# gattia/pyfocusr

Measured on AMD Instinct MI355X. Metric: lowest-k eigenpairs/sec + KNN-correspondence wall-clock, 250k-vertex mesh pair k=5, higher is better.
Workload: dtype f64

## Files before the change

### include/pyfocusr_hip.h

```cpp
#ifndef PYFOCUSR_HIP_H
#define PYFOCUSR_HIP_H

#include <stddef.h>
#include <stdint.h>

#ifdef __cplusplus
extern "C" {
#endif

#define PF_VERSION 1

#define PF_OK 0
#define PF_E_ARG (-1)
#define PF_E_HIP (-2)
#define PF_E_DEGENERATE (-3)
#define PF_E_STATE (-4)
#define PF_E_PERSIST_TIMEOUT (-5)

#define PF_OP_RW 0
#define PF_OP_SYM 1

typedef struct pf_ctx pf_ctx;
typedef struct pf_graph pf_graph;
typedef struct pf_mesh pf_mesh;

typedef struct pf_graph_info {
    int64_t n;
    int64_t n_faces;
    int64_t nnz_w;
    int64_t nnz_l;
    int32_t is_symmetric;
    int32_t n_isolated;
    int32_t n_components;
    int32_t max_degree;
    int64_t sell_entries;
    int64_t n_pad;
    int64_t n_oneway;
    double spectral_bound;
} pf_graph_info;

typedef struct pf_timing {
    double op_ms;
    int64_t op_launches;
    double op_bytes;
    double knn_ms;
    double build_ms;
    double persist_ms;
    int64_t persist_launches;
    int64_t persist_steps;
    double persist_bytes;
    double persist_lds_bytes;
} pf_timing;

int pf_version(void);
const char* pf_last_error(void);
int pf_device_count(void);
int pf_create(int device, pf_ctx** out);
void pf_destroy(pf_ctx* ctx);
int pf_sync(pf_ctx* ctx);
void* pf_stream(pf_ctx* ctx);
int pf_timing_enable(pf_ctx* ctx, int on);
int pf_timing_get(pf_ctx* ctx, pf_timing* out, int reset);

int pf_graph_build(pf_ctx* ctx, const double* pts, int64_t n, const int32_t* faces, int64_t n_faces,
                   int32_t verts_per_face, pf_graph** out);
int pf_mesh_upload(pf_ctx* ctx, const double* pts, int64_t n, const int32_t* faces, int64_t n_faces,
                   int32_t verts_per_face, pf_mesh** out);
void pf_mesh_free(pf_mesh* mesh);
int pf_graph_build_device(pf_mesh* mesh, pf_graph** out);
int pf_graph_build_device2(pf_mesh* mesh_a, pf_mesh* mesh_b, pf_graph** out_a, pf_graph** out_b);
int pf_graph_from_matrix(pf_ctx* ctx, int64_t n, const int32_t* rowptr, const int32_t* colidx, const double* values,
                         pf_graph** out);
void pf_graph_free(pf_graph* g);
int pf_graph_get_info(pf_graph* g, pf_graph_info* out);
int pf_graph_download(pf_graph* g, int32_t* rowptr, int32_t* colidx, double* w, double* l_offdiag,
                      double* deg, double* l_diag, int32_t* component_label);

int pf_ws_ensure(pf_graph* g, int32_t n_slots);
int pf_ws_upload(pf_graph* g, int32_t slot, const double* x);
int pf_ws_download(pf_graph* g, int32_t first, int32_t count, double* out);
int pf_ws_copy(pf_graph* g, int32_t src, int32_t dst, int32_t count);
int pf_start_vector(pf_graph* g, int32_t slot, uint64_t seed);
int pf_mask_isolated(pf_graph* g, int32_t slot);
int pf_lock_null_vectors(pf_graph* g, int32_t op, int32_t* n_locked);

int pf_spmv(pf_graph* g, int32_t op, int32_t src, int32_t dst);
int pf_spmv_multi(pf_graph* g, int32_t op, int32_t src_first, int32_t dst_first, int32_t count);
int pf_persist_enable(int on);
int pf_persist_two_step(int level);
int pf_persist_pair_halves(int on);
int pf_persist_clock(pf_ctx* ctx, double* kernel_ms, int64_t* launches, int reset);
typedef struct pf_persist_info {
    int32_t enabled;
    int32_t two_step;
    int32_t owner;
    int32_t timeouts;
    int64_t launches;
    int64_t launches_two_step;
    int32_t suspended_for;
    int32_t rearms;
    int32_t owner_switches;
    int32_t hold_ticks;
} pf_persist_info;
int pf_persist_state(pf_ctx* ctx , pf_persist_info* out);
int pf_persist_test_hook(int n_launches);
int pf_cheb(pf_graph* g, int32_t op, int32_t src, int32_t dst, int32_t degree, double c, double e, double rho);
int pf_cheb2(pf_graph* ga, int32_t op_a, int32_t src_a, int32_t dst_a, int32_t degree_a, double c_a, double e_a, double rho_a,
             pf_graph* gb, int32_t op_b, int32_t src_b, int32_t dst_b, int32_t degree_b, double c_b, double e_b, double rho_b);
int pf_dots(pf_graph* g, int32_t w, int32_t first, int32_t count, double* out);
int pf_orth(pf_graph* g, int32_t w, int32_t first, int32_t count, double* h, double* nrm);
int pf_orth_begin(pf_graph* g, int32_t w, int32_t first, int32_t count, int32_t normalize);
int pf_orth_end(pf_graph* g, double* h, double* nrm);
int pf_orth_begin2(pf_graph* ga, int32_t w_a, int32_t first_a, int32_t count_a, int32_t normalize_a, pf_graph* gb, int32_t w_b,
                   int32_t first_b, int32_t count_b, int32_t normalize_b);
int pf_orth_cheb2(pf_graph* ga, pf_graph* gb, const int32_t* orth, const int32_t* cheb_i, const double* cheb_d);
int pf_orth_redone(pf_graph* g);
int pf_orth_strict(pf_graph* g, int32_t on);
int pf_orth_device_passes(pf_graph* g, int32_t on);
int pf_orth_split(pf_graph* g, int32_t first2, int32_t split);
int pf_orth_one_launch(int32_t on);
int pf_scale(pf_graph* g, int32_t slot, double alpha);
int pf_combine(pf_graph* g, int32_t src_first, int32_t m, const double* Y, int32_t k, int32_t dst_first);
int pf_resnorm(pf_graph* g, int32_t ax, int32_t x, double lam, double* out);
int pf_gram(pf_graph* g, int32_t first_a, int32_t count_a, int32_t first_b, int32_t count_b, double* out);
int pf_resnorms(pf_graph* g, int32_t ax_first, int32_t x_first, const double* lam, int32_t count, double* out);
int pf_finalize_vectors(pf_graph* g, int32_t first, int32_t count, int32_t from_sym, int32_t minmax,
                        double* out);
int pf_finalize_vectors_begin(pf_graph* g, int32_t first, int32_t count, int32_t from_sym, int32_t minmax, double* out);
int pf_finalize_vectors_end(pf_graph* g);
int pf_final_remap_begin(pf_graph* g, const int32_t* col, const double* sign, int32_t count, double* out);
int pf_host_alloc(size_t bytes, void** out);
int pf_host_free(void* p);
int pf_host_detach(void* p);
int pf_final_rows(pf_graph* g, const int64_t* rows, int64_t n_rows, double* out);
int pf_point_rows(pf_graph* g, const int64_t* rows, int64_t n_rows, double* out);
int pf_spmv_host(pf_graph* g, int32_t op, const double* x, double* y);
int pf_mean_filter(pf_graph* g, const double* values, int32_t ncols, int32_t iterations, double* out);

int pf_knn1(pf_ctx* ctx, const double* ref, int64_t n_ref, const double* qry, int64_t n_qry, int32_t d,
            int64_t* idx_out, double* d2_out);
int pf_knn_mode(pf_ctx* ctx, int32_t mode);
int pf_knn_tree_stats(pf_ctx* ctx, int32_t enable_counting, int64_t* leaves_scanned, int64_t* supers_opened);
int pf_knn_count(pf_ctx* ctx, int32_t enable_counting, int64_t* pairs);
int pf_knn_wave_stats(pf_ctx* ctx, double* sum_us, double* max_us, int64_t* waves, int64_t* max_candidates, double* detail);
int pf_knn(pf_ctx* ctx, const double* ref, int64_t n_ref, const double* qry, int64_t n_qry, int32_t d, int32_t k,
           int64_t* idx_out, double* d2_out);
int pf_knn1_graphs(pf_graph* ref_g, pf_graph* qry_g, int32_t d, const int32_t* col_ref, const double* scale_ref,
                   const int32_t* col_qry, const double* scale_qry, int64_t* idx_out, double* d2_out);
int pf_knn1_blocks(pf_ctx* ctx, const double* ref_block, int64_t n_ref, int32_t ref_stride, const double* qry_block,
                   int64_t n_qry, int32_t qry_stride, int32_t d, const int32_t* col_ref, const double* scale_ref,
                   const int32_t* col_qry, const double* scale_qry, int64_t* idx_out, double* d2_out);
int pf_eigsort_costs(pf_graph* g_target, pf_graph* g_source, const int64_t* rows_t, int64_t m_t, const int64_t* rows_s, int64_t m_s,
                     int32_t k, const int32_t* col_t, const double* sign_t, const int32_t* col_s, const double* sign_s, double* out,
                     int64_t* idx_out);
int pf_final_device(pf_graph* g, double** block, int64_t* n_rows, int32_t* n_cols);
int pf_knn_upload(pf_ctx* ctx, const double* ref, int64_t n_ref, const double* qry, int64_t n_qry, int32_t d);
int pf_knn_run(pf_ctx* ctx);
int pf_knn_download(pf_ctx* ctx, int64_t* idx_out, double* d2_out);

typedef struct pf_eigs_stats {
    int64_t matvecs;
    int32_t outer_steps;
    int32_t restarts;
    int32_t filter_resets;
    int32_t degree;
    int32_t n_null;
    double cut;
    double max_residual;
    int32_t second_passes;
    int32_t mode;
    int32_t local_steps;
    int32_t reserved;
} pf_eigs_stats;
int pf_eigs_smallest(pf_graph* g, int32_t n_wanted, int32_t minmax, double* vals, double* vecs, int32_t* n_out,
                     pf_eigs_stats* stats);
int pf_eigs_smallest_ex(pf_graph* g, int32_t n_wanted, int32_t minmax, int32_t async_download, double* vals, double* vecs,
                        double* residuals, int32_t* n_out, pf_eigs_stats* stats);
int pf_eigs_smallest2(pf_graph* ga, pf_graph* gb, int32_t n_wanted_a, int32_t n_wanted_b, int32_t minmax, int32_t async_download,
                      double* vals_a, double* vecs_a, double* res_a, int32_t* n_out_a, pf_eigs_stats* stats_a,
                      double* vals_b, double* vecs_b, double* res_b, int32_t* n_out_b, pf_eigs_stats* stats_b);

typedef struct pf_rows pf_rows;
int pf_op_step(pf_graph* g, int32_t op, int32_t x, int32_t prev, int32_t out, double alpha, double shift, double beta);
int pf_cheb_steps(pf_graph* g, int32_t op, int32_t prev, int32_t cur, int32_t k_first, int32_t n_steps, double c, double e,
                  double rho, int32_t* out_prev, int32_t* out_cur);
int pf_axpy(pf_graph* g, int32_t w, int32_t first, int32_t count, const double* coef);
int pf_rows_create(pf_graph* g, const int64_t* rows, int64_t n, pf_rows** out);
void pf_rows_free(pf_rows* r);
int pf_rows_gather(pf_rows* r, int32_t slot, double* out);
int pf_rows_scatter(pf_rows* r, int32_t slot, const double* in);
int pf_rows_gather_dev(pf_rows* r, int32_t slot, double* dst_device);
int pf_rows_scatter_dev(pf_rows* r, int32_t slot, const double* src_device);
int pf_rows_set_sources(pf_rows* r, const int64_t* offsets);
int pf_rows_gather2_dev(pf_rows* r, int32_t slot_a, int32_t slot_b, double* dst_device, int64_t stride);
int pf_rows_scatter2_dev(pf_rows* r, int32_t slot_a, int32_t slot_b, const double* src_device, int64_t stride);
int pf_rows_fill(pf_rows* r, int32_t slot, double value);

typedef struct pf_surface pf_surface;
int pf_surface_create(pf_ctx* ctx, const double* points, int64_t n, const int32_t* faces, int64_t n_faces,
                      int32_t verts_per_face, pf_surface** out);
void pf_surface_free(pf_surface* s);
int pf_surface_closest(pf_surface* s, const double* qry, int64_t n_qry, double* out_pts, int32_t* out_face,
                       double* out_d2);
int pf_surface_distance(pf_surface* s, const double* qry, int64_t n_qry, double* out_d2, int32_t* out_face,
                        double* stats);
int pf_surface_prepare_signed(pf_surface* s, const double* points, const int32_t* faces, int64_t* topology);
int pf_surface_signed_distance(pf_surface* s, const double* qry, int64_t n_qry, double* out_sd, int32_t* out_face,
                               int32_t* out_feature, int64_t* n_ambiguous);
int pf_surface_prepare_winding(pf_surface* s);
int pf_surface_winding(pf_surface* s, const double* qry, int64_t n_qry, double beta, double* out_w, double* out_bound);

typedef struct pf_cpd pf_cpd;
int pf_cpd_create(pf_ctx* ctx, const double* X, int64_t N, const double* Y, int64_t M, int32_t d, pf_cpd** out);
void pf_cpd_free(pf_cpd* h);
int pf_cpd_estep(pf_cpd* h, const double* TY, double sigma2, double w, double* P1, double* Pt1, double* PX);
int pf_cpd_set_basis(pf_cpd* h, const double* Q, int32_t K);
int pf_cpd_weighted_gram(pf_cpd* h, double* H);
int pf_cpd_affine_sums(pf_cpd* h, double* shifts, double* sums);
int pf_cpd_apply_affine(pf_cpd* h, const double* B, const double* t);
int pf_cpd_deform_sums(pf_cpd* h, double* H, double* R);
int pf_cpd_apply_deform(pf_cpd* h, const double* C, double* sums);
int pf_cpd_download(pf_cpd* h, double* TY, double* P1, double* Pt1, double* PX);
int pf_cpd_gram(pf_ctx* ctx, const double* A, int64_t n_a, const double* B, int64_t n_b, int32_t d, double beta,
                const double* V, int32_t n_cols, double* out);

typedef struct pf_assign_stats {
    int32_t phases;
    int32_t dense_passes;
    int64_t rounds;
    int64_t bids;
    int64_t dense_bids;
// ... 19 lines not shown
```

### pyfocusr_amd/_hip.py

```python
import atexit
import ctypes as C
import os
import threading
import weakref

import numpy as np

_HERE = os.path.dirname(os.path.abspath(__file__))
LIB_PATH = os.environ.get("PYFOCUSR_HIP_LIB", os.path.join(_HERE, "csrc", "libpyfocusr_hip.so"))

PF_OP_RW = 0
PF_OP_SYM = 1

_f64p = C.POINTER(C.c_double)
_i32p = C.POINTER(C.c_int32)
_i64p = C.POINTER(C.c_int64)


class HipUnavailable(RuntimeError):
    pass


class PfError(RuntimeError):
    def __init__(self, code, msg):
        RuntimeError.__init__(self, "libpyfocusr_hip error %d: %s" % (code, msg))
        self.code = code


class GraphInfo(C.Structure):
    _fields_ = [("n", C.c_int64), ("n_faces", C.c_int64), ("nnz_w", C.c_int64), ("nnz_l", C.c_int64),
                ("is_symmetric", C.c_int32), ("n_isolated", C.c_int32), ("n_components", C.c_int32),
                ("max_degree", C.c_int32), ("sell_entries", C.c_int64), ("n_pad", C.c_int64), ("n_oneway", C.c_int64),
                ("spectral_bound", C.c_double)]


class EigsStats(C.Structure):
    _fields_ = [("matvecs", C.c_int64), ("outer_steps", C.c_int32), ("restarts", C.c_int32), ("filter_resets", C.c_int32),
                ("degree", C.c_int32), ("n_null", C.c_int32), ("cut", C.c_double), ("max_residual", C.c_double),
                ("second_passes", C.c_int32), ("mode", C.c_int32), ("local_steps", C.c_int32), ("reserved", C.c_int32)]


class Timing(C.Structure):
    _fields_ = [("op_ms", C.c_double), ("op_launches", C.c_int64), ("op_bytes", C.c_double), ("knn_ms", C.c_double),
                ("build_ms", C.c_double), ("persist_ms", C.c_double), ("persist_launches", C.c_int64),
                ("persist_steps", C.c_int64), ("persist_bytes", C.c_double), ("persist_lds_bytes", C.c_double)]


class AssignStats(C.Structure):
    _fields_ = [("phases", C.c_int32), ("dense_passes", C.c_int32), ("rounds", C.c_int64), ("bids", C.c_int64),
                ("dense_bids", C.c_int64), ("candidate_edges", C.c_int64), ("launches", C.c_int64),
                ("device_bytes", C.c_int64), ("k", C.c_int32), ("eps_floor_hit", C.c_int32), ("eps_initial", C.c_double),
                ("eps_final", C.c_double), ("eps_floor", C.c_double), ("total_cost", C.c_double),
                ("gap_bound", C.c_double), ("lower_bound", C.c_double), ("ms_candidates", C.c_double),
                ("ms_auction", C.c_double), ("ms_certificate", C.c_double)]

    def as_dict(self):
        return {name: getattr(self, name) for name, _ in self._fields_}


SIGNATURES = {
    "pf_version": (C.c_int, []),
    "pf_last_error": (C.c_char_p, []),
    "pf_device_count": (C.c_int, []),
    "pf_create": (C.c_int, [C.c_int, C.POINTER(C.c_void_p)]),
    "pf_destroy": (None, [C.c_void_p]),
    "pf_sync": (C.c_int, [C.c_void_p]),
    "pf_stream": (C.c_void_p, [C.c_void_p]),
    "pf_timing_enable": (C.c_int, [C.c_void_p, C.c_int]),
    "pf_timing_get": (C.c_int, [C.c_void_p, C.POINTER(Timing), C.c_int]),
    "pf_graph_build": (C.c_int, [C.c_void_p, _f64p, C.c_int64, _i32p, C.c_int64, C.c_int32, C.POINTER(C.c_void_p)]),
    "pf_mesh_upload": (C.c_int, [C.c_void_p, _f64p, C.c_int64, _i32p, C.c_int64, C.c_int32, C.POINTER(C.c_void_p)]),
    "pf_mesh_free": (None, [C.c_void_p]),
    "pf_graph_build_device": (C.c_int, [C.c_void_p, C.POINTER(C.c_void_p)]),
    "pf_graph_build_device2": (C.c_int, [C.c_void_p, C.c_void_p, C.POINTER(C.c_void_p), C.POINTER(C.c_void_p)]),
    "pf_graph_from_matrix": (C.c_int, [C.c_void_p, C.c_int64, _i32p, _i32p, _f64p, C.POINTER(C.c_void_p)]),
    "pf_graph_free": (None, [C.c_void_p]),
    "pf_graph_get_info": (C.c_int, [C.c_void_p, C.POINTER(GraphInfo)]),
    "pf_graph_download": (C.c_int, [C.c_void_p, _i32p, _i32p, _f64p, _f64p, _f64p, _f64p, _i32p]),
    "pf_ws_ensure": (C.c_int, [C.c_void_p, C.c_int32]),
    "pf_ws_upload": (C.c_int, [C.c_void_p, C.c_int32, _f64p]),
    "pf_ws_download": (C.c_int, [C.c_void_p, C.c_int32, C.c_int32, _f64p]),
    "pf_ws_copy": (C.c_int, [C.c_void_p, C.c_int32, C.c_int32, C.c_int32]),
    "pf_start_vector": (C.c_int, [C.c_void_p, C.c_int32, C.c_uint64]),
    "pf_mask_isolated": (C.c_int, [C.c_void_p, C.c_int32]),
    "pf_lock_null_vectors": (C.c_int, [C.c_void_p, C.c_int32, _i32p]),
    "pf_spmv": (C.c_int, [C.c_void_p, C.c_int32, C.c_int32, C.c_int32]),
    "pf_spmv_multi": (C.c_int, [C.c_void_p, C.c_int32, C.c_int32, C.c_int32, C.c_int32]),
    "pf_knn_mode": (C.c_int, [C.c_void_p, C.c_int32]),
    "pf_knn_tree_stats": (C.c_int, [C.c_void_p, C.c_int32, C.POINTER(C.c_int64), C.POINTER(C.c_int64)]),
    "pf_persist_enable": (C.c_int, [C.c_int]),
    "pf_persist_two_step": (C.c_int, [C.c_int]),
    "pf_persist_pair_halves": (C.c_int, [C.c_int]),
    "pf_persist_clock": (C.c_int, [C.c_void_p, C.POINTER(C.c_double), C.POINTER(C.c_int64), C.c_int]),
    "pf_persist_state": (C.c_int, [C.c_void_p, C.c_void_p]),
    "pf_persist_test_hook": (C.c_int, [C.c_int]),
    "pf_cheb": (C.c_int, [C.c_void_p, C.c_int32, C.c_int32, C.c_int32, C.c_int32, C.c_double, C.c_double, C.c_double]),
    "pf_cheb2": (C.c_int, [C.c_void_p, C.c_int32, C.c_int32, C.c_int32, C.c_int32, C.c_double, C.c_double, C.c_double,
                           C.c_void_p, C.c_int32, C.c_int32, C.c_int32, C.c_int32, C.c_double, C.c_double, C.c_double]),
    "pf_dots": (C.c_int, [C.c_void_p, C.c_int32, C.c_int32, C.c_int32, _f64p]),
    "pf_orth": (C.c_int, [C.c_void_p, C.c_int32, C.c_int32, C.c_int32, _f64p, _f64p]),
    "pf_orth_begin": (C.c_int, [C.c_void_p, C.c_int32, C.c_int32, C.c_int32, C.c_int32]),
    "pf_orth_end": (C.c_int, [C.c_void_p, _f64p, _f64p]),
    "pf_orth_split": (C.c_int, [C.c_void_p, C.c_int32, C.c_int32]),
    "pf_orth_one_launch": (C.c_int, [C.c_int32]),
    "pf_orth_begin2": (C.c_int, [C.c_void_p, C.c_int32, C.c_int32, C.c_int32, C.c_int32, C.c_void_p, C.c_int32, C.c_int32, C.c_int32,
                                 C.c_int32]),
    "pf_orth_cheb2": (C.c_int, [C.c_void_p, C.c_void_p, _i32p, _i32p, _f64p]),
    "pf_eigsort_costs": (C.c_int, [C.c_void_p, C.c_void_p, _i64p, C.c_int64, _i64p, C.c_int64, C.c_int32, _i32p, _f64p, _i32p, _f64p, _f64p,
                                   _i64p]),
    "pf_orth_redone": (C.c_int, [C.c_void_p]),
    "pf_orth_strict": (C.c_int, [C.c_void_p, C.c_int32]),
    "pf_scale": (C.c_int, [C.c_void_p, C.c_int32, C.c_double]),
    "pf_combine": (C.c_int, [C.c_void_p, C.c_int32, C.c_int32, _f64p, C.c_int32, C.c_int32]),
    "pf_resnorm": (C.c_int, [C.c_void_p, C.c_int32, C.c_int32, C.c_double, _f64p]),
    "pf_gram": (C.c_int, [C.c_void_p, C.c_int32, C.c_int32, C.c_int32, C.c_int32, _f64p]),
    "pf_resnorms": (C.c_int, [C.c_void_p, C.c_int32, C.c_int32, _f64p, C.c_int32, _f64p]),
    "pf_finalize_vectors": (C.c_int, [C.c_void_p, C.c_int32, C.c_int32, C.c_int32, C.c_int32, _f64p]),
    "pf_finalize_vectors_begin": (C.c_int, [C.c_void_p, C.c_int32, C.c_int32, C.c_int32, C.c_int32, _f64p]),
    "pf_finalize_vectors_end": (C.c_int, [C.c_void_p]),
    "pf_final_remap_begin": (C.c_int, [C.c_void_p, _i32p, _f64p, C.c_int32, _f64p]),
    "pf_host_alloc": (C.c_int, [C.c_size_t, C.POINTER(C.c_void_p)]),
    "pf_host_free": (C.c_int, [C.c_void_p]),
    "pf_final_rows": (C.c_int, [C.c_void_p, _i64p, C.c_int64, _f64p]),
    "pf_point_rows": (C.c_int, [C.c_void_p, _i64p, C.c_int64, _f64p]),
    "pf_spmv_host": (C.c_int, [C.c_void_p, C.c_int32, _f64p, _f64p]),
    "pf_mean_filter": (C.c_int, [C.c_void_p, _f64p, C.c_int32, C.c_int32, _f64p]),
    "pf_knn1": (C.c_int, [C.c_void_p, _f64p, C.c_int64, _f64p, C.c_int64, C.c_int32, _i64p, _f64p]),
    "pf_knn": (C.c_int, [C.c_void_p, _f64p, C.c_int64, _f64p, C.c_int64, C.c_int32, C.c_int32, _i64p, _f64p]),
    "pf_knn1_graphs": (C.c_int, [C.c_void_p, C.c_void_p, C.c_int32, _i32p, _f64p, _i32p, _f64p, _i64p, _f64p]),
    "pf_knn1_blocks": (C.c_int, [C.c_void_p, C.c_void_p, C.c_int64, C.c_int32, C.c_void_p, C.c_int64, C.c_int32, C.c_int32,
                                 _i32p, _f64p, _i32p, _f64p, _i64p, _f64p]),
    "pf_final_device": (C.c_int, [C.c_void_p, C.POINTER(C.c_void_p), _i64p, _i32p]),
    "pf_knn_upload": (C.c_int, [C.c_void_p, _f64p, C.c_int64, _f64p, C.c_int64, C.c_int32]),
    "pf_knn_run": (C.c_int, [C.c_void_p]),
    "pf_knn_download": (C.c_int, [C.c_void_p, _i64p, _f64p]),
    "pf_eigs_smallest": (C.c_int, [C.c_void_p, C.c_int32, C.c_int32, _f64p, _f64p, C.POINTER(C.c_int32), C.POINTER(EigsStats)]),
    "pf_knn_count": (C.c_int, [C.c_void_p, C.c_int32, C.POINTER(C.c_int64)]),
    "pf_knn_wave_stats": (C.c_int, [C.c_void_p, C.POINTER(C.c_double), C.POINTER(C.c_double), C.POINTER(C.c_int64), C.POINTER(C.c_int64),
                                    _f64p]),
    "pf_host_detach": (C.c_int, [C.c_void_p]),
    "pf_orth_device_passes": (C.c_int, [C.c_void_p, C.c_int32]),
    "pf_eigs_smallest_ex": (C.c_int, [C.c_void_p, C.c_int32, C.c_int32, C.c_int32, _f64p, _f64p, _f64p, C.POINTER(C.c_int32),
                                      C.POINTER(EigsStats)]),
    "pf_eigs_smallest2": (C.c_int, [C.c_void_p, C.c_void_p, C.c_int32, C.c_int32, C.c_int32, C.c_int32,
                                    _f64p, _f64p, _f64p, C.POINTER(C.c_int32), C.POINTER(EigsStats),
                                    _f64p, _f64p, _f64p, C.POINTER(C.c_int32), C.POINTER(EigsStats)]),
    "pf_op_step": (C.c_int, [C.c_void_p, C.c_int32, C.c_int32, C.c_int32, C.c_int32, C.c_double, C.c_double, C.c_double]),
    "pf_cheb_steps": (C.c_int, [C.c_void_p, C.c_int32, C.c_int32, C.c_int32, C.c_int32, C.c_int32, C.c_double, C.c_double,
                                C.c_double, C.POINTER(C.c_int32), C.POINTER(C.c_int32)]),
    "pf_axpy": (C.c_int, [C.c_void_p, C.c_int32, C.c_int32, C.c_int32, _f64p]),
    "pf_rows_create": (C.c_int, [C.c_void_p, _i64p, C.c_int64, C.POINTER(C.c_void_p)]),
    "pf_rows_free": (None, [C.c_void_p]),
    "pf_rows_gather": (C.c_int, [C.c_void_p, C.c_int32, _f64p]),
    "pf_rows_scatter": (C.c_int, [C.c_void_p, C.c_int32, _f64p]),
    "pf_rows_gather_dev": (C.c_int, [C.c_void_p, C.c_int32, C.c_void_p]),
    "pf_rows_scatter_dev": (C.c_int, [C.c_void_p, C.c_int32, C.c_void_p]),
    "pf_rows_set_sources": (C.c_int, [C.c_void_p, _i64p]),
    "pf_rows_gather2_dev": (C.c_int, [C.c_void_p, C.c_int32, C.c_int32, C.c_void_p, C.c_int64]),
    "pf_rows_scatter2_dev": (C.c_int, [C.c_void_p, C.c_int32, C.c_int32, C.c_void_p, C.c_int64]),
    "pf_rows_fill": (C.c_int, [C.c_void_p, C.c_int32, C.c_double]),
    "pf_surface_create": (C.c_int, [C.c_void_p, _f64p, C.c_int64, _i32p, C.c_int64, C.c_int32, C.POINTER(C.c_void_p)]),
    "pf_surface_free": (None, [C.c_void_p]),
    "pf_surface_closest": (C.c_int, [C.c_void_p, _f64p, C.c_int64, _f64p, _i32p, _f64p]),
    "pf_surface_distance": (C.c_int, [C.c_void_p, _f64p, C.c_int64, _f64p, _i32p, _f64p]),
    "pf_surface_prepare_signed": (C.c_int, [C.c_void_p, _f64p, _i32p, _i64p]),
    "pf_surface_signed_distance": (C.c_int, [C.c_void_p, _f64p, C.c_int64, _f64p, _i32p, _i32p, _i64p]),
    "pf_surface_prepare_winding": (C.c_int, [C.c_void_p]),
    "pf_surface_winding": (C.c_int, [C.c_void_p, _f64p, C.c_int64, C.c_double, _f64p, _f64p]),
    "pf_cpd_create": (C.c_int, [C.c_void_p, _f64p, C.c_int64, _f64p, C.c_int64, C.c_int32, C.POINTER(C.c_void_p)]),
    "pf_cpd_free": (None, [C.c_void_p]),
    "pf_cpd_estep": (C.c_int, [C.c_void_p, _f64p, C.c_double, C.c_double, _f64p, _f64p, _f64p]),
    "pf_cpd_set_basis": (C.c_int, [C.c_void_p, _f64p, C.c_int32]),
    "pf_cpd_weighted_gram": (C.c_int, [C.c_void_p, _f64p]),
    "pf_cpd_affine_sums": (C.c_int, [C.c_void_p, _f64p, _f64p]),
    "pf_cpd_apply_affine": (C.c_int, [C.c_void_p, _f64p, _f64p]),
    "pf_cpd_deform_sums": (C.c_int, [C.c_void_p, _f64p, _f64p]),
    "pf_cpd_apply_deform": (C.c_int, [C.c_void_p, _f64p, _f64p]),
    "pf_cpd_download": (C.c_int, [C.c_void_p, _f64p, _f64p, _f64p, _f64p]),
    "pf_cpd_gram": (C.c_int, [C.c_void_p, _f64p, C.c_int64, _f64p, C.c_int64, C.c_int32, C.c_double, _f64p, C.c_int32, _f64p]),
    "pf_assign": (C.c_int, [C.c_void_p, _f64p, C.c_int64, _f64p, C.c_int64, C.c_int32, _i64p, _f64p, _f64p,
                            C.POINTER(AssignStats)]),
}

_lib = None
_lib_lock = threading.Lock()
_live_graphs = weakref.WeakSet()
_live_contexts = weakref.WeakSet()


@atexit.register
def _shutdown():
    for g in list(_live_graphs):
        g.close()
    for c in list(_live_contexts):
        c.close()


def load_library():
    global _lib
    with _lib_lock:
        if _lib is not None:
            return _lib
        if not os.path.exists(LIB_PATH):
            raise HipUnavailable(
                "%s not found: build it with `python -c 'import __graft_entry__ as g; g.build()'` "
                "(hipcc --offload-arch=gfx950); there is no CPU fallback" % LIB_PATH)
        lib = C.CDLL(LIB_PATH)
        for name, (res, args) in SIGNATURES.items():
            fn = getattr(lib, name)
            fn.restype = res
            fn.argtypes = args
        _lib = lib
        return lib


PF_E_DEGENERATE = -3
PF_E_STATE = -4
PF_E_PERSIST_TIMEOUT = -5


class _PinnedBlock(object):
    __slots__ = ("ptr", "nbytes")

    def __init__(self, ptr, nbytes):
        self.ptr, self.nbytes = ptr, nbytes

    def __del__(self):
        try:
            _pinned_release(self.ptr, self.nbytes)
        except Exception:
            pass

# ... 856 lines not shown
```

### pyfocusr_amd/csrc/pf_assemble.hip

```cpp
#include <string.h>

#include <algorithm>
#include <string>

#include "pf_internal.h"
#include "pf_launch.h"

namespace {

struct k_count_edges {
    static constexpr int BOUNDS = PF_BLOCK;
    static __device__ __forceinline__ void run(const int32_t* __restrict__ faces, int64_t n_edges,
                                                          int32_t vpf, int64_t n, int32_t* __restrict__ cnt,
                                                          int32_t* __restrict__ rank, int32_t* __restrict__ flags,
                                                          double* __restrict__ quarter) {
    const int64_t e = (int64_t)blockIdx.x * PF_BLOCK + threadIdx.x;
    if (e == 0 && quarter) *quarter = 0.25;
    if (e >= n_edges) return;
    const int64_t f = e / vpf;
    const int32_t k = (int32_t)(e - f * vpf);
    const int32_t src = faces[e];
    const int32_t dst = faces[f * vpf + (k + 1 == vpf ? 0 : k + 1)];
    if (src < 0 || src >= n || dst < 0 || dst >= n) {
        atomicOr(flags, 1);
// ... 814 lines not shown
            PF_TRY(scratch(&b_rank, n_edges));
            PF_TRY(scratch(&b_start, n + 1));
            PF_TRY(scratch(&b_rcol, n_edges));
            PF_TRY(scratch(&b_rw, n_edges));
            PF_TRY(dev_alloc(st, &g->rowptr, n + 1));
            PF_TRY(dev_alloc(st, &g->deg, 3 * g->n_pad));
            g->g = g->deg + g->n_pad;
            g->sg = g->deg + 2 * g->n_pad;
            g->deg_block = true;
            PF_TRY(dev_alloc(st, &g->diag, g->n_pad));
            PF_TRY(dev_alloc(st, &g->label, g->n_pad));
            PF_TRY(dev_alloc(st, &g->perm, g->n_pad));
            PF_TRY(dev_alloc(st, &g->iperm, g->n_pad));
            PF_TRY(dev_alloc(st, &g->smooth, g->n_pad));
            PF_TRY(dev_alloc(st, &g->slice_ptr, g->n_slices + 1));

            PF_TRY(dev_alloc(st, &g->perm_m, g->n_pad));
            PF_TRY(dev_alloc(st, &g->iperm_m, g->n_pad));
            PF_HIP(pfl::memset_words(st, zeroed, 0, sizeof(int32_t) * (size_t)(2 * zstride + 8)));
            PF_HIP(pfl::memset_words(st, g->deg, 0, sizeof(double) * 3 * g->n_pad));
            if (pos == 0) PF_HIP(pfl::event_record(st, ctx->ev0));
            PF_TRY(pf_morton_order(g, mesh->pts, robust ? nullptr : b_flags + 1));
            PF_TRY(scratch(&pts_m, 3 * n));
            PF_TRY(scratch(&faces_m, n_edges));
            d_pts = pts_m, d_faces = faces_m;
            if (n) {
                pfl::launch<k_renumber_points>(dim3(nblk(3 * n)), dim3(PF_BLOCK), 0, st, mesh->pts, g->morder, n, pts_m);
                PF_HIP(hipGetLastError());
            }
            if (n_edges) {
                pfl::launch<k_renumber_faces>(dim3(nblk(n_edges)), dim3(PF_BLOCK), 0, st, mesh->faces, g->mrank, n_edges, n, faces_m);
                PF_HIP(hipGetLastError());
            }

            if (face_bound) PF_TRY(scratch(&pmin, 1));
            if (n_edges) {
                pfl::launch<k_count_edges>(dim3(nblk(n_edges)), dim3(PF_BLOCK), 0, st, d_faces, n_edges, vpf, n, b_cnt, b_rank, b_flags, reinterpret_cast<double*>(pmin));
                PF_HIP(hipGetLastError());
            }
            PF_TRY(pf_exclusive_scan_i32(st, b_cnt, b_start, n + 1));
            if (n_edges) {
                pfl::launch<k_scatter_edges>(dim3(nblk(n_edges)), dim3(PF_BLOCK), 0, st, d_faces, d_pts, n_edges, vpf, n, b_start, b_rank, b_rcol, b_rw, b_flags);
                PF_HIP(hipGetLastError());
            }
            return PF_OK;
        }
        if (k == 1) {
            pfl::launch<k_sort_unique_rows>(dim3(nblk(n)), dim3(PF_BLOCK), 0, st, b_start, n, b_rcol, b_rw, b_ucnt, g->morder);
            PF_HIP(hipGetLastError());
            PF_TRY(pf_exclusive_scan_i32(st, b_ucnt, g->rowptr, n + 1));
            PF_TRY(dev_alloc(st, &g->col, n_edges));
            PF_TRY(dev_alloc(st, &g->w, n_edges));
            pfl::launch<k_compact_rows>(dim3(nblk(n)), dim3(PF_BLOCK), 0, st, b_start, g->rowptr, n, b_rcol, b_rw, g->col, g->w, g->deg, g->g, g->sg);
            PF_HIP(hipGetLastError());
            if (pfl::tl_rec && pf_stream_b(ctx) && ctx->fork_ev) {
                hipStream_t side = ctx->stream_b;
                hipEvent_t ev = ctx->fork_ev;
                pfl::call(st, [=](hipStream_t s) {
                    (void)hipEventRecord(ev, s);
                    (void)hipStreamWaitEvent(side, ev, 0);
                });
                g->side_stream = side;
            }
            if (face_bound) {
                pfl::launch<k_face_bound>(dim3(nblk(n_faces)), dim3(PF_BLOCK), 0, g->side_stream ? g->side_stream : st, d_faces, d_pts, n_faces, n, pmin);
                PF_HIP(hipGetLastError());
            }
            fin.g = g, fin.d_pts = d_pts, fin.numeric_symmetry = false, fin.d_extra = b_flags, fin.h_extra = h_flags;
            fin.nnz_from_rowptr = true, fin.d_pmin = pmin, fin.h_pmin = &h_pmin, fin.pos = pos;
            return PF_OK;
        }
        if (k == 2) return fin.begin_stats_and_labels();
        return fin.queue_order(false);
    }

    int end() {
        const int64_t n = mesh->n;
        PF_TRY(fin.end());
        if (h_flags[1] != 0 && !(h_flags[0] & 7)) {
            needs_robust = true;
            return PF_OK;
        }
        PF_CHECK(!(h_flags[0] & 1), PF_E_ARG, "pf_graph_build: face index out of range [0,%lld)", (long long)n);
        PF_CHECK(!(h_flags[0] & 2), PF_E_DEGENERATE, "pf_graph_build: a face repeats a vertex on one edge");
        PF_CHECK(!(h_flags[0] & 4), PF_E_DEGENERATE,
                 "pf_graph_build: an edge has zero length or non-finite coordinates (the reference would store an "
                 "infinite weight, graph.py:177-178)");
        PF_CHECK(!fin.extra_hit, PF_E_HIP, "pf_graph_build: unexpected assembly flag");
        g->spectral_bound = 2.0;
        if (pmin && g->is_symmetric && g->nnz_w == n_edges && h_pmin > 0.0 && h_pmin <= 0.25) {
            const double disc = 1.0 - 4.0 * h_pmin;
            const double b = (1.0 + (1.0 + sqrt(disc > 0.0 ? disc : 0.0)) / 2.0) * (1.0 + 1e-12);
            g->spectral_bound = b < 2.0 ? b : 2.0;
        }
        PF_TRY(dev_alloc(st, &g->pts, 3 * n));
        PF_HIP(pfl::memcpy_async(st, g->pts, mesh->pts, sizeof(double) * 3 * n, hipMemcpyDeviceToDevice));
        return PF_OK;
    }
};

}

extern "C" {

void pf_graph_free(pf_graph* g) {
    if (!g) return;
    if (!g->ctx) {
        delete g;
        return;
    }
    hipSetDevice(g->ctx->device);
    hipStream_t st = g->ctx->stream;
    (void)pf_finalize_vectors_end(g);
    {
        std::lock_guard<std::mutex> lk(g->ctx->deferred_mutex);
        auto& dq = g->ctx->deferred;
        dq.erase(std::remove(dq.begin(), dq.end(), g), dq.end());
    }
    if (g->final_stats) g->ctx->pinned_pool.emplace_back(g->final_stats_cap, reinterpret_cast<double*>(g->final_stats));
    if (g->final_ready) g->ctx->event_pool.push_back(g->final_ready);
    if (g->final_done) g->ctx->event_pool.push_back(g->final_done);
    pf_free(st, g->persist_ring);
    pf_free(st, g->persist_ring2);
    pf_free(st, g->final_vecs);
    pf_free(st, g->pts);
    pf_window_slots_free(g);
    pf_free(st, g->rowptr);
    pf_free(st, g->col);
    pf_free(st, g->w);
    pf_free(st, g->deg);
    if (!g->deg_block) {
        pf_free(st, g->g);
        pf_free(st, g->sg);
    }
    pf_free(st, g->label);
    if (g->perm_m != g->perm) pf_free(st, g->perm_m);
    if (g->iperm_m != g->iperm) pf_free(st, g->iperm_m);
    pf_free(st, g->morder);
    pf_free(st, g->mrank);
    pf_free(st, g->order_bbox);
    pf_free(st, g->perm);
    pf_free(st, g->iperm);
    pf_free(st, g->smooth);
    pf_free(st, g->stage);
    pf_free(st, g->slice_ptr);
    pf_free(st, g->scol);
    pf_free(st, g->sval_rw);
    pf_free(st, g->sval_sym);
    pf_free(st, g->diag);
    pf_free(st, g->mf_col);
    pf_free(st, g->mf_val);
    pf_free(st, g->ws);
    pf_free(st, g->partials);
    pf_free(st, g->coef);
    pf_free(st, g->orth_counter);
    if (g->orth_pending >= 0 || g->small_pending > 0 || g->px_state == -2) pfl::sync(st);
    if (g->orth_host) g->ctx->pinned_pool.emplace_back(g->orth_host_cap, g->orth_host);
    if (g->orth_ev) g->ctx->event_pool.push_back(g->orth_ev);
    if (g->px_host) g->ctx->pinned_pool.emplace_back(g->px_host_cap, g->px_host);
    if (g->px_ev) g->ctx->event_pool.push_back(g->px_ev);
    if (g->small_host) g->ctx->pinned_pool.emplace_back(g->small_host_cap, g->small_host);
    if (g->small_ev) g->ctx->event_pool.push_back(g->small_ev);
    delete g;
}


int pf_mesh_upload(pf_ctx* ctx, const double* pts, int64_t n, const int32_t* faces, int64_t n_faces, int32_t vpf,
                   pf_mesh** out) {
    PF_CHECK(ctx && pts && out && (faces || n_faces == 0), PF_E_ARG, "pf_mesh_upload: NULL argument");
    PF_CHECK(n > 0 && n < (int64_t)1 << 31, PF_E_ARG, "pf_mesh_upload: n = %lld out of range", (long long)n);
    PF_CHECK(n_faces >= 0 && vpf >= 2 && n_faces * vpf < (int64_t)1 << 31, PF_E_ARG,
             "pf_mesh_upload: faces %lld x %d out of range", (long long)n_faces, vpf);
    *out = nullptr;
    PF_HIP(hipSetDevice(ctx->device));
    pf_mesh* m = new pf_mesh();
    m->ctx = ctx;
    m->n = n;
    m->n_faces = n_faces;
    m->vpf = vpf;
    hipStream_t st = ctx->stream;
    int r = dev_alloc(st, &m->pts, 3 * n);
    if (r == PF_OK) r = dev_alloc(st, &m->faces, n_faces * vpf);
    hipError_t e = hipSuccess;
    if (r == PF_OK) e = pfl::memcpy_async(ctx->stream, m->pts, pts, sizeof(double) * 3 * n, hipMemcpyHostToDevice);
    if (r == PF_OK && e == hipSuccess && n_faces)
        e = pfl::memcpy_async(ctx->stream, m->faces, faces, sizeof(int32_t) * n_faces * vpf, hipMemcpyHostToDevice);
    if (r == PF_OK && e == hipSuccess) e = pfl::sync(ctx->stream);
    if (r != PF_OK || e != hipSuccess) {
        if (e != hipSuccess) pf_set_error("pf_mesh_upload: %s", hipGetErrorString(e));
        pf_mesh_free(m);
        return r != PF_OK ? r : PF_E_HIP;
    }
    *out = m;
    return PF_OK;
}

void pf_mesh_free(pf_mesh* m) {
    if (!m) return;
    pf_free(m->ctx->stream, m->pts);
    pf_free(m->ctx->stream, m->faces);
    delete m;
}

int pf_graph_build(pf_ctx* ctx, const double* pts, int64_t n, const int32_t* faces, int64_t n_faces,
                   int32_t vpf, pf_graph** out) {
    PF_CHECK(out != nullptr, PF_E_ARG, "pf_graph_build: out is NULL");
    *out = nullptr;
    pf_mesh* m = nullptr;
    PF_TRY(pf_mesh_upload(ctx, pts, n, faces, n_faces, vpf, &m));
    int r = pf_graph_build_device(m, out);
    pf_mesh_free(m);
    return r;
}

int pf_graph_build_device(pf_mesh* mesh, pf_graph** out) {
    PF_CHECK(mesh && out, PF_E_ARG, "pf_graph_build_device: NULL argument");
    pf_ctx* ctx = mesh->ctx;
    *out = nullptr;
    PF_HIP(hipSetDevice(ctx->device));
    MeshBuild job;
    PF_TRY(job.begin(mesh));
    PF_TRY(job.end());
    if (job.needs_robust) {
        if (getenv("PF_DEBUG_WINDOWS")) fprintf(stderr, "pyfocusr_hip: renumbering by counting gave up, building again with the general sort\n");
        MeshBuild again;
        again.robust = true;
        PF_TRY(again.begin(mesh));
        PF_TRY(again.end());
        PF_HIP(pfl::sync(ctx->stream));
        again.ok = true;
        *out = again.g;
        return PF_OK;
    }
    PF_HIP(pfl::event_record(ctx->stream, ctx->ev1));
    ctx->build_pending = true;
    if (pf_persist_enabled()) PF_TRY(pf_window_slots_begin(job.g));
    job.ok = true;
    *out = job.g;
    return PF_OK;
}

int pf_graph_build_device2(pf_mesh* mesh_a, pf_mesh* mesh_b, pf_graph** out_a, pf_graph** out_b) {
    PF_CHECK(mesh_a && mesh_b && out_a && out_b, PF_E_ARG, "pf_graph_build_device2: NULL argument");
    PF_CHECK(mesh_a->ctx == mesh_b->ctx, PF_E_ARG, "pf_graph_build_device2: the two meshes must belong to one ctx");
    pf_ctx* ctx = mesh_a->ctx;
    *out_a = *out_b = nullptr;
    PF_HIP(hipSetDevice(ctx->device));
    if (!pf_stream_b(ctx)) {
        PF_TRY(pf_graph_build_device(mesh_a, out_a));
        const int r = pf_graph_build_device(mesh_b, out_b);
        if (r != PF_OK) {
            pf_graph_free(*out_a);
            *out_a = nullptr;
        }
        return r;
    }
    hipStream_t st = ctx->stream;
    bool redo = false;
    {
        MeshBuild a, b;
        pfl::Recorder ra, rb;
        struct Unhook {
            ~Unhook() { pfl::tl_rec = nullptr; }
        } unhook;
        int rc = a.prepare(mesh_a, 0);
        if (rc == PF_OK) rc = b.prepare(mesh_b, 1);
        for (int k = 0; k < MeshBuild::N_PHASES && rc == PF_OK; ++k) {
            pfl::tl_rec = &ra;
            rc = a.phase(k);
            pfl::tl_rec = &rb;
            if (rc == PF_OK) rc = b.phase(k);
            pfl::tl_rec = nullptr;
            pfl::flush(ra, &rb);
        }
        if (rc == PF_OK) {
            pfl::tl_rec = &ra;
            rc = a.end();
            pfl::tl_rec = &rb;
            if (rc == PF_OK) rc = b.end();
            if (rc == PF_OK && !(a.needs_robust || b.needs_robust) && pf_persist_enabled()) {
                pfl::tl_rec = &ra;
                rc = pf_window_slots_begin(a.g);
                pfl::tl_rec = &rb;
                if (rc == PF_OK) rc = pf_window_slots_begin(b.g);
            }
        }
        pfl::tl_rec = nullptr;
        pfl::flush(ra, &rb);
        if (rc != PF_OK) {
            (void)pfl::sync(ctx->stream_b);
            (void)pfl::sync(st);
        }
        a.release();
        b.release();
        if (rc == PF_OK) {
            const hipError_t e1 = hipEventRecord(ctx->ev1, st);
            if (e1 == hipSuccess) ctx->build_pending = true;
            else rc = PF_E_HIP, pf_set_error("pf_graph_build_device2: %s", hipGetErrorString(e1));
        }
        if (rc != PF_OK) return rc;
        if (a.needs_robust || b.needs_robust) {
            redo = true;
        } else {
            a.ok = b.ok = true;
            *out_a = a.g;
            *out_b = b.g;
// ... 208 lines not shown
```

### pyfocusr_amd/csrc/pf_eigs.hip

```cpp
#include <math.h>

#include <algorithm>
#include <vector>

#include "pf_internal.h"
#include "pf_krylov.h"

namespace {

struct DeviceOps final : pfk::Ops {
    pf_graph* g;
    explicit DeviceOps(pf_graph* graph) : g(graph) {}
    int64_t n() const override { return g->n; }
    int64_t n_isolated() const override { return g->n_isolated; }
    int32_t n_components() const override { return g->n_components; }
    int32_t n_oneway() const override { return g->n_oneway; }
    bool symmetric() const override { return g->is_symmetric; }
    double spectral_bound() const override { return g->spectral_bound; }
    int ws_ensure(int32_t slots) override { return pf_ws_ensure(g, slots); }
    int lock_nulls(int32_t op, int32_t* locked) override { return pf_lock_null_vectors(g, op, locked); }
    int orth_strict(bool on) override { return pf_orth_strict(g, on ? 1 : 0); }
    int orth_always_twice(bool on, bool strict_otherwise) override { return pf_orth_strict(g, on ? 2 : (strict_otherwise ? 1 : 0)); }
    int orth_device_passes(bool on) override { return pf_orth_device_passes(g, on ? 1 : 0); }
    int start_vector(int32_t slot, uint64_t seed) override { return pf_start_vector(g, slot, seed); }
    int orth_begin(int32_t w, int32_t first, int32_t count) override { return pf_orth_begin(g, w, first, count, 1); }
    int orth_end(double* h, double* nrm, bool* redone) override {
        PF_TRY(pf_orth_end(g, h, nrm));
        const int r = pf_orth_redone(g);
        *redone = r == 1;
        last_twice = r == 2;
        return PF_OK;
    }
    int cheb(int32_t op, int32_t src, int32_t dst, int32_t degree, double c, double e, double rho) override {
        return pf_cheb(g, op, src, dst, degree, c, e, rho);
    }
    int combine(int32_t src_first, int32_t m, const double* Y, int32_t k, int32_t dst_first) override {
        return pf_combine(g, src_first, m, Y, k, dst_first);
    }
    int combine2(int32_t src_first, int32_t m, const double* Y, int32_t k, int32_t dst_first, int32_t src_first2, int32_t dst_first2) override {
        return pf_combine2(g, src_first, m, Y, k, dst_first, src_first2, dst_first2);
    }
    int copy(int32_t src, int32_t dst, int32_t count) override { return pf_ws_copy(g, src, dst, count); }
    int spmv_multi(int32_t op, int32_t src_first, int32_t dst_first, int32_t count) override {
        return pf_spmv_multi(g, op, src_first, dst_first, count);
    }
    int gram(int32_t first_a, int32_t count_a, int32_t first_b, int32_t count_b, double* out) override {
        return pf_gram(g, first_a, count_a, first_b, count_b, out);
    }
    int resnorms(int32_t ax_first, int32_t x_first, const double* lam, int32_t count, double* out) override {
        return pf_resnorms(g, ax_first, x_first, lam, count, out);
    }
    int gram_begin(int32_t first_a, int32_t count_a, int32_t first_b, int32_t count_b, bool self_b) override {
        PF_TRY(pf_gram_begin(g, first_a, count_a, first_b, count_b, 0));
        return self_b ? pf_gram_begin(g, first_b, count_b, first_b, count_b, 1) : PF_OK;
    }
    bool orth_split(int32_t first2, int32_t split) override { return pf_orth_split(g, first2, split) == PF_OK; }
    int gram_end(double* out) override { return pf_small_end(g, out); }
    int resnorms_begin(int32_t ax_first, int32_t x_first, const double* lam, int32_t count) override {
        return pf_resnorms_begin(g, ax_first, x_first, lam, count);
    }
    int resnorms_end(double* out) override { return pf_small_end(g, out); }
    int orth_begin_pair(pfk::Ops& other, const int32_t* o) override {
        return pf_orth_begin2(g, o[0], o[1], o[2], o[3], static_cast<DeviceOps&>(other).g, o[4], o[5], o[6], o[7]);
    }
    int cheb_pair(pfk::Ops& other, const int32_t* ci, const double* cd) override {
        return pf_cheb2(g, ci[0], ci[1], ci[2], ci[3], cd[0], cd[1], cd[2], static_cast<DeviceOps&>(other).g, ci[4], ci[5], ci[6], ci[7], cd[3],
                        cd[4], cd[5]);
    }
    int orth_cheb_pair(pfk::Ops& other, const int32_t* orth, const int32_t* ci, const double* cd) override {
        return pf_orth_cheb2(g, static_cast<DeviceOps&>(other).g, orth, ci, cd);
    }
};

int ellipse_hint() {
    const char* ev = getenv("PF_EIGS_ELLIPSE");
    return ev ? atoi(ev) : -1;
}

void give_up(pf_graph* g) {
    if (!g) return;
    if (g->orth_pending >= 0) {
        std::vector<double> h((size_t)g->orth_pending + 1);
        double nrm = 0.0;
        (void)pf_orth_end(g, h.data(), &nrm);
    }
    if (g->small_pending > 0) {
        (void)hipEventSynchronize(g->small_ev);
        g->small_pending = 0;
    }
    (void)pf_download_cancel(g);
}

int finish(pf_graph* g, pfk::Solver& s, int32_t minmax, double* vals, double* vecs, double* residuals, int32_t* n_out, pf_eigs_stats* stats,
           bool async) {
    *n_out = s.n_out;
    for (int i = 0; i < s.n_out; ++i) {
        vals[i] = s.vals[(size_t)i];
        if (residuals) residuals[i] = s.residuals[(size_t)i];
    }
    if (stats) *stats = s.st;
    if (s.n_out > 0) {
        PF_TRY(pf_finalize_vectors_begin(g, s.first_slot, s.n_out, s.sym ? 1 : 0, minmax ? 1 : 0, vecs));
        if (!async) PF_TRY(pf_finalize_vectors_end(g));
    }
    return PF_OK;
}

}

extern "C" int pf_eigs_smallest_ex(pf_graph* g, int32_t n_wanted, int32_t minmax, int32_t async_download, double* vals, double* vecs,
                                   double* residuals, int32_t* n_out, pf_eigs_stats* stats_out) {
    PF_CHECK(g && vals && vecs && n_out && n_wanted >= 1, PF_E_ARG, "pf_eigs_smallest: bad argument");
    int rc = PF_OK;
    for (int attempt = 0; attempt < 3; ++attempt) {
        DeviceOps ops(g);
        pfk::Solver s;
        *n_out = 0;
        rc = s.init(&ops, n_wanted, ellipse_hint());
        if (rc == PF_OK) rc = pfk::drive_single(s);
        if (rc == PF_OK) rc = pf_sync(g->ctx);
        if (rc == PF_OK) rc = finish(g, s, minmax, vals, vecs, residuals, n_out, stats_out, async_download != 0);
        if (rc != PF_OK) give_up(g);
        if (rc != PF_E_PERSIST_TIMEOUT) break;
    }
    return rc;
}

extern "C" int pf_eigs_smallest(pf_graph* g, int32_t n_wanted, int32_t minmax, double* vals, double* vecs, int32_t* n_out,
                                pf_eigs_stats* stats_out) {
    return pf_eigs_smallest_ex(g, n_wanted, minmax, 0, vals, vecs, nullptr, n_out, stats_out);
}

extern "C" int pf_eigs_smallest2(pf_graph* ga, pf_graph* gb, int32_t n_wanted_a, int32_t n_wanted_b, int32_t minmax, int32_t async_download,
                                 double* vals_a, double* vecs_a, double* res_a, int32_t* n_out_a, pf_eigs_stats* stats_a,
                                 double* vals_b, double* vecs_b, double* res_b, int32_t* n_out_b, pf_eigs_stats* stats_b) {
    PF_CHECK(ga && gb && ga != gb && vals_a && vecs_a && n_out_a && vals_b && vecs_b && n_out_b && n_wanted_a >= 1 && n_wanted_b >= 1,
             PF_E_ARG, "pf_eigs_smallest2: bad argument");
    PF_CHECK(ga->ctx == gb->ctx, PF_E_ARG, "pf_eigs_smallest2: the two graphs must share one ctx (stream)");
    int rc = PF_OK;
    for (int attempt = 0; attempt < 3; ++attempt) {
        DeviceOps oa(ga), ob(gb);
        pfk::Solver a, b;
        *n_out_a = *n_out_b = 0;
        rc = a.init(&oa, n_wanted_a, ellipse_hint());
        if (rc == PF_OK) rc = b.init(&ob, n_wanted_b, ellipse_hint());
        if (rc == PF_OK) rc = pfk::drive_pair(a, b);
        if (rc == PF_OK) rc = pf_sync(ga->ctx);
        if (rc == PF_OK) rc = finish(ga, a, minmax, vals_a, vecs_a, res_a, n_out_a, stats_a, async_download != 0);
        if (rc == PF_OK) rc = finish(gb, b, minmax, vals_b, vecs_b, res_b, n_out_b, stats_b, async_download != 0);
        if (rc != PF_OK) {
            give_up(ga);
            give_up(gb);
        }
        if (rc != PF_E_PERSIST_TIMEOUT) break;
    }
    return rc;
}
```

### pyfocusr_amd/csrc/pf_internal.h

```cpp
#pragma once
#include <hip/hip_runtime.h>
#include <stdint.h>
#include <atomic>
#include <map>
#include <mutex>
#include <unordered_map>
#include <vector>

#include "../../include/pyfocusr_hip.h"

void pf_set_error(const char* fmt, ...);

#define PF_HIP(call)                                                                          \
    do {                                                                                      \
        hipError_t e_ = (call);                                                               \
        if (e_ != hipSuccess) {                                                               \
            pf_set_error("%s:%d %s: %s", __FILE__, __LINE__, #call, hipGetErrorString(e_));   \
            (void)hipGetLastError();  \
            return PF_E_HIP;                                                                  \
        }                                                                                     \
    } while (0)

#define PF_CHECK(cond, code, ...)        \
    do {                                 \
// ... 36 lines not shown

struct pf_ctx {
    int device = 0;
    hipStream_t stream = nullptr;
    void* stage_ring = nullptr;
    hipEvent_t stage_ev[8] = {nullptr, nullptr, nullptr, nullptr, nullptr, nullptr, nullptr, nullptr};
    int stage_next = 0;
    hipStream_t copy_stream = nullptr;
    hipEvent_t ev0 = nullptr, ev1 = nullptr;
    bool timing = false;
    int timing_stride = 1;
    int64_t timing_count = 0;
    uint32_t* persist_sync = nullptr;
    int32_t* persist_abort = nullptr;
    void* persist_cal = nullptr;
    double op_ms = 0.0;
    int64_t op_launches = 0;
    double op_bytes = 0.0;
    double persist_ms = 0.0, persist_bytes = 0.0, persist_lds_bytes = 0.0;
    int64_t persist_launches = 0, persist_steps = 0;
    double knn_ms = 0.0;
    double build_ms = 0.0;
    bool build_pending = false;
    double* knn_ref = nullptr;
    double* knn_qry = nullptr;
    double* knn_ref_s = nullptr;
    double* knn_ref_soa = nullptr;
    int64_t knn_cap_ref_soa = 0, knn_ref_ld = 0;
    double* knn_qry_s = nullptr;
    unsigned* knn_ref_key = nullptr;
    unsigned* knn_qry_key = nullptr;
    int32_t* knn_cell_start = nullptr;
    int64_t knn_cap_cell = 0;
    int knn_res = 0;
    void* knn_grid = nullptr;
    int32_t* knn_ref_orig = nullptr;
    int32_t* knn_qry_orig = nullptr;
    unsigned long long* knn_ext = nullptr;
    int64_t knn_nref = 0, knn_nqry = 0;
    int64_t knn_cap_ref = 0, knn_cap_qry = 0, knn_cap_ref_s = 0, knn_cap_qry_s = 0, knn_cap_ref_key = 0,
            knn_cap_qry_key = 0, knn_cap_ref_orig = 0, knn_cap_qry_orig = 0, knn_cap_idx = 0, knn_cap_d2 = 0;
    int32_t knn_d = 0;
    int32_t knn_k = 1, knn_k_next = 1;
    int64_t* knn_idx = nullptr;
    double* knn_d2 = nullptr;
    bool knn_ready = false, knn_done = false;
    pf_knn_tree knn_tree;
    bool knn_count_on = false;
    unsigned long long* knn_visited = nullptr;
    size_t knn_visited_words = 0;
    int64_t knn_visited_waves = 0;
    int32_t knn_mode = 0;
    struct TimedSpan {
        hipEvent_t e0, e1;
        int64_t launches;
        double bytes;
        int64_t persist_steps;
        double lds_bytes;
    };
    std::vector<TimedSpan> spans_pending;
    std::vector<std::pair<hipEvent_t, hipEvent_t>> spans_free;
    std::vector<std::pair<int32_t, double*>> pinned_pool;
    void* pinned_scratch = nullptr;
    size_t pinned_scratch_bytes = 0;
    std::vector<hipEvent_t> event_pool;
    std::multimap<size_t, void*> free_blocks;
    std::unordered_map<void*, size_t> live_blocks;
    std::mutex alloc_mutex;
    hipStream_t stream_b = nullptr;
    hipEvent_t join_ev = nullptr, fork_ev = nullptr;
    std::vector<pf_graph*> deferred;
    std::mutex deferred_mutex;
    int64_t alloc_misses = 0;
    void* pinned_scratch_b = nullptr;
    size_t pinned_scratch_b_bytes = 0;
    void* pinned_scratch_knn = nullptr;
    size_t pinned_scratch_knn_bytes = 0;
};

inline uint64_t pf_next_uid() {
    static std::atomic<uint64_t> next{1};
    return next.fetch_add(1);
}

struct pf_graph {
    hipStream_t side_stream = nullptr;
    uint64_t uid = pf_next_uid();
    pf_ctx* ctx = nullptr;
    int64_t n = 0, n_pad = 0, n_faces = 0;
    int32_t vpf = 0;
    int32_t* rowptr = nullptr;
    int32_t* col = nullptr;
    double* w = nullptr;
    int64_t nnz_w = 0;
    double* deg = nullptr;
    double* g = nullptr;
    double* sg = nullptr;
    int32_t* label = nullptr;
    int32_t* morder = nullptr;
    int32_t* mrank = nullptr;
    int32_t* perm_m = nullptr;
    int32_t* iperm_m = nullptr;
    int32_t* perm = nullptr;
    int32_t* iperm = nullptr;
    unsigned long long* order_bbox = nullptr;
    double* smooth = nullptr;
    double* stage = nullptr;
    int64_t stage_cap = 0;
    int64_t n_slices = 0, sell_entries = 0;
    int64_t* slice_ptr = nullptr;
    int32_t* scol = nullptr;
    double* sval_rw = nullptr;
    double* sval_sym = nullptr;
    double* diag = nullptr;
    int32_t* mf_col = nullptr;
    double* mf_val = nullptr;
    int32_t win_rows = 1024;
    std::vector<int64_t> h_slice_ptr;
    int32_t px_state = -1;
    double* px_host = nullptr;
    int32_t px_host_cap = 0;
    hipEvent_t px_ev = nullptr;
    int32_t* px_slot = nullptr;
    int32_t* px_gh_cnt = nullptr;
    int32_t* px_gh_row = nullptr;
    int32_t* px_need = nullptr;
    std::vector<int32_t> h_px_gh_cnt;
    int64_t px_gh_total = 0;
    double* persist_ring = nullptr;
    int32_t persist_phase = 0;
    uint64_t persist_epoch = 0;
    int32_t px2_state = -1;
    int32_t* px_gh_cnt2 = nullptr;
    int32_t* px_need2 = nullptr;
    uint8_t* px_g1_w = nullptr;
    int32_t* px_g1_pos = nullptr;
    uint16_t* px_g1_slot = nullptr;
    int32_t* px_g1_gw = nullptr;
    std::vector<int32_t> h_px_gh_cnt2, h_px_g1_gw;
    int64_t px_gh2_total = 0, px_g1_entries = 0;
    int32_t single_applications = 0;
    uint64_t lds_need_partner = 0;
    int64_t lds_need_value = -2, lds_need2_value = -2;
    double* persist_ring2 = nullptr;
    int32_t persist_phase2 = 0;
    uint64_t persist_epoch2 = 0;
    int32_t is_symmetric = 0, n_isolated = 0, n_components = 0, max_degree = 0, n_oneway = 0;
    int32_t unit_g = 0;
    std::vector<int32_t> roots;
    double* ws = nullptr;
    int32_t n_slots = 0;
    double* partials = nullptr;
    int32_t partial_cap = 0;
    double* coef = nullptr;
    int32_t coef_cap = 0;
    int64_t n_chunks = 0;
    double* orth_host = nullptr;
    int32_t orth_host_cap = 0;
    int32_t orth_pending = -1;
    hipEvent_t orth_ev = nullptr;
    double* small_host = nullptr;
    int32_t small_host_cap = 0, small_pending = 0;
    bool small_root = false;
    hipEvent_t small_ev = nullptr;
    hipEvent_t orth_wait = nullptr;
    int32_t orth_w = 0, orth_first = 0, orth_normalize = 0;
    int32_t orth_redone = 0;
    double orth_serial = 0.0;
    unsigned long long* orth_counter = nullptr;
    unsigned long long orth_arrivals = 0;
    uint64_t orth_epoch = 0;
    int32_t orth_split = -1, orth_first2 = 0;
    int32_t orth_split_now = -1, orth_first2_now = 0;
    double orth_ticket = 0.0;
    double orth_thresh = 0.09;
    int32_t orth_device_passes = 0;
    int32_t orth_twice = 0;
    double* final_vecs = nullptr;
    int32_t final_count = 0;
    int32_t final_pending = 0;
    double* final_params = nullptr;
    void* final_stats = nullptr;
    int32_t final_stats_cap = 0;
    hipEvent_t final_ready = nullptr, final_done = nullptr;
    const double* dl_src = nullptr;
    double* dl_dst = nullptr;
    size_t dl_bytes = 0;
    int32_t final_check = 0;
    double* final_tmp = nullptr;
    double* pts = nullptr;
    bool deg_block = false;
    double spectral_bound = 2.0;
};

int pf_timing_collect(pf_ctx* c);
hipError_t pf_malloc(hipStream_t st, void** p, size_t bytes);
int pf_pinned_scratch(pf_ctx* c, size_t bytes, void** out, int which = 0);
int pf_copy_by_kernel(hipStream_t st, const void* src, void* dst, size_t bytes);
int pf_downloads_release(pf_ctx* c);
int pf_download_cancel(pf_graph* g);
hipStream_t pf_stream_b(pf_ctx* c);
hipError_t pf_create_side_stream(hipStream_t* s, bool low = false);
void pf_free(hipStream_t st, void* p);

__host__ __device__ static inline int64_t pf_sell_index(int64_t base, int32_t width, int32_t j, int lane) {
    const int32_t pairs = width >> 1;
    return j < 2 * pairs ? base + (int64_t)(j >> 1) * (2 * PF_WAVE) + 2 * lane + (j & 1)
                         : base + (int64_t)pairs * (2 * PF_WAVE) + lane;
}

static inline double* pf_slot(pf_graph* g, int32_t s) { return g->ws + (int64_t)s * g->n_pad; }
static inline double* pf_tmp(pf_graph* g, int which) { return g->ws + (int64_t)(g->n_slots + which) * g->n_pad; }

int pf_exclusive_scan_i32(hipStream_t st, const int32_t* in, int32_t* out, int64_t n);
int pf_exclusive_scan_i64(hipStream_t st, const int64_t* in, int64_t* out, int64_t n);

int pf_reduce_ensure(pf_graph* g, int32_t count);

int pf_compute_order(pf_graph* g, const double* d_pts, int32_t* d_overflow = nullptr);
int pf_morton_order(pf_graph* g, const double* d_pts, int32_t* d_overflow);

static inline int32_t pf_window_rows(int64_t n_pad) { return n_pad <= 262144 ? 1024 : (n_pad <= 524288 ? 2048 : 4096); }

constexpr int PF_KNN_TREE_MIN_D = 7;
int pf_knn_tree_run(pf_ctx* c);

int pf_gram_begin(pf_graph* g, int32_t first_a, int32_t count_a, int32_t first_b, int32_t count_b, int32_t append);
int pf_resnorms_begin(pf_graph* g, int32_t ax_first, int32_t x_first, const double* lam, int32_t count);
int pf_small_end(pf_graph* g, double* out);
int pf_combine2(pf_graph* g, int32_t src_first, int32_t m, const double* Y, int32_t k, int32_t dst_first, int32_t src_first2,
                int32_t dst_first2);

struct pf_persist_args {
    pf_graph* g;
    const double* vals;
    const double* src;
    double* dst;
    int32_t degree;
    double c, e, rho;
};
int pf_persist_cheb(const pf_persist_args* a, const pf_persist_args* b , int* done, double* lds_bytes ,
                    bool first_try = true );
int pf_persist_check(pf_ctx* ctx);
int pf_persist_set(int on);
void pf_persist_release(pf_ctx* ctx);
int pf_window_slots_prepare(pf_graph* g);
int pf_window_slots_begin(pf_graph* g);
bool pf_persist_enabled();
bool pf_persist_trusted();
uint64_t pf_persist_abort_epoch();
int pf_persist_sync_ensure(pf_ctx* ctx);
int pf_window_rings_prepare(pf_graph* g);
void pf_window_slots_free(pf_graph* g);
```

### pyfocusr_amd/csrc/pf_operator.hip

```cpp
#include <math.h>
#include <stdlib.h>
#include <string.h>

#include <algorithm>
#include <atomic>
#include <map>
#include <mutex>
#include <vector>

#include "pf_internal.h"

namespace {

inline unsigned nblk(int64_t n) { return (unsigned)((n + PF_BLOCK - 1) / PF_BLOCK); }

#ifndef PF_OP_BLOCK
#define PF_OP_BLOCK 256
#endif
struct OpArgs {
    const int64_t* slice_ptr;
    const int32_t* scol;
    const double* sval;
    const double* diag;
    const double* x;
// ... 388 lines not shown
                           (unsigned long long)__double_as_longlong(p), __ATOMIC_RELAXED, __HIP_MEMORY_SCOPE_AGENT);
        asm volatile("s_waitcnt vmcnt(0)" ::: "memory");
    }
    __syncthreads();
    if (threadIdx.x == 0) s_ok = orth_meet(a, a.target);
    __syncthreads();
    if (!s_ok) return;
    {
        const int b0 = threadIdx.x / PF_WAVE, b1 = b0 + PF_BLOCK / PF_WAVE;
        double s0 = 0.0, s1 = 0.0;
        for (int64_t k = lane; k < a.n_chunks; k += PF_WAVE) {
            const double x0 = b0 < count + 1 ? __longlong_as_double((long long)__hip_atomic_load(
                                                   reinterpret_cast<unsigned long long*>(a.partial) + (int64_t)b0 * a.n_chunks + k, __ATOMIC_RELAXED,
                                                   __HIP_MEMORY_SCOPE_AGENT))
                                             : 0.0;
            const double x1 = b1 < count + 1 ? __longlong_as_double((long long)__hip_atomic_load(
                                                   reinterpret_cast<unsigned long long*>(a.partial) + (int64_t)b1 * a.n_chunks + k, __ATOMIC_RELAXED,
                                                   __HIP_MEMORY_SCOPE_AGENT))
                                             : 0.0;
            s0 += x0;
            s1 += x1;
        }
#pragma unroll
        for (int off = PF_WAVE / 2; off > 0; off >>= 1) {
            s0 += __shfl_down(s0, off, PF_WAVE);
            s1 += __shfl_down(s1, off, PF_WAVE);
        }
        if (lane == 0 && b0 < count + 1) hs[b0] = s0;
        if (lane == 0 && b1 < count + 1) hs[b1] = s1;
    }
    __syncthreads();
    if (threadIdx.x == 0) {
        double sum = 0.0;
        for (int b = 0; b < count; ++b) sum += hs[b] * hs[b];
        const double before = hs[count], after = before - sum;
        int fine = after >= a.thresh * before ? 1 : 0;
        asm volatile("" : "+v"(fine));
        s_redo = fine ? 0.0 : 1.0;
        s_after = after;
        s_scale = (fine && a.normalize && after > 1e-280) ? 1.0 / sqrt(after) : 1.0;
    }
    __syncthreads();
    if (chunk == 0) {
        for (int b = threadIdx.x; b < count; b += PF_BLOCK) {
            a.hsum[b] = hs[b];
            a.host_out[b] = hs[b];
        }
        if (threadIdx.x == 0) {
            *a.nrm2 = s_after;
            a.host_out[count] = s_after;
            a.host_out[count + 1] = s_redo;
        }
        __threadfence_system();
        __syncthreads();
        if (threadIdx.x == 0) __hip_atomic_store(a.host_out + count + 2, a.ticket, __ATOMIC_RELEASE, __HIP_MEMORY_SCOPE_SYSTEM);
    }
    const double sc = s_scale;
#pragma unroll
    for (int it = 0; it < PAIRS; ++it) {
        double2 acc = cs[it];
#pragma unroll
        for (int u = 0; u < PF_ORTH_LOCAL_MAX; ++u) {
            if (u >= count) continue;
            const double hb = hs[u];
            acc.x -= hb * xs[u][it].x;
            acc.y -= hb * xs[u][it].y;
        }
        acc.x *= sc;
        acc.y *= sc;
        *reinterpret_cast<double2*>(w + lo + 2 * threadIdx.x + (int64_t)it * (2 * PF_BLOCK)) = acc;
    }
}
__global__ __launch_bounds__(PF_BLOCK) void k_scale_finishing(double* __restrict__ x, int64_t n_pad, const double* __restrict__ partial,
                                                              int64_t n_chunks, int normalize, const double* __restrict__ hsum,
                                                              int32_t count, double* __restrict__ nrm2, double* __restrict__ host_out) {
    __shared__ double s_v;
    if (threadIdx.x < PF_WAVE) {
        double s = 0.0;
        for (int64_t k = threadIdx.x; k < n_chunks; k += PF_WAVE) s += partial[k];
#pragma unroll
        for (int off = PF_WAVE / 2; off > 0; off >>= 1) s += __shfl_down(s, off, PF_WAVE);
        if (threadIdx.x == 0) s_v = s;
    }
    __syncthreads();
    const double v = s_v;
    if (blockIdx.x == 0) {
        for (int b = threadIdx.x; b < count; b += PF_BLOCK) host_out[b] = hsum[b];
        if (threadIdx.x == 0) {
            *nrm2 = v;
            host_out[count] = v;
            host_out[count + 1] = 0.0;
        }
    }
    const int64_t i = (int64_t)blockIdx.x * PF_BLOCK + threadIdx.x;
    if (normalize && i < n_pad && v > 1e-280) x[i] *= 1.0 / sqrt(v);
}

__global__ __launch_bounds__(PF_BLOCK) void k_scale(double* __restrict__ x, int64_t n_pad, double alpha) {
    const int64_t i = (int64_t)blockIdx.x * PF_BLOCK + threadIdx.x;
    if (i < n_pad) x[i] *= alpha;
}

__global__ __launch_bounds__(PF_BLOCK) void k_scale_rsqrt(double* __restrict__ x, int64_t n_pad, const double* __restrict__ nrm2) {
    const int64_t i = (int64_t)blockIdx.x * PF_BLOCK + threadIdx.x;
    const double v = *nrm2;
    if (i < n_pad && v > 1e-280) x[i] *= 1.0 / sqrt(v);
}

__global__ __launch_bounds__(PF_BLOCK) void k_mask_isolated(double* __restrict__ x, const int32_t* __restrict__ rowptr,
                                                            const int32_t* __restrict__ perm, int64_t n) {
    const int64_t r = (int64_t)blockIdx.x * PF_BLOCK + threadIdx.x;
    if (r >= n) return;
    const int32_t i = perm[r];
    if (rowptr[i + 1] == rowptr[i]) x[r] = 0.0;
}

__global__ __launch_bounds__(PF_BLOCK) void k_start_vector(double* __restrict__ x, const double* __restrict__ smooth,
                                                           const int32_t* __restrict__ perm, const int32_t* __restrict__ perm_m,
                                                           const int32_t* __restrict__ rowptr,
                                                           int64_t n_pad, unsigned long long seed, double noise) {
    const int64_t r = (int64_t)blockIdx.x * PF_BLOCK + threadIdx.x;
    if (r >= n_pad) return;
    const int32_t i = perm[r];
    const int32_t m = perm_m[r];
    double v = 0.0;
    if (i >= 0 && rowptr[m + 1] > rowptr[m]) {
        unsigned long long z = seed + 0x9E3779B97F4A7C15ull * (unsigned long long)(i + 1);
        z = (z ^ (z >> 30)) * 0xBF58476D1CE4E5B9ull;
        z = (z ^ (z >> 27)) * 0x94D049BB133111EBull;
        z ^= z >> 31;
        const double u = (double)(z >> 11) * (1.0 / 9007199254740992.0) - 0.5;
        v = smooth[r] + noise * u;
    }
    x[r] = v;
}

__global__ __launch_bounds__(PF_BLOCK) void k_permute_in(const double* __restrict__ src_old, const int32_t* __restrict__ perm,
                                                         int64_t n_pad, double* __restrict__ dst_new) {
    const int64_t r = (int64_t)blockIdx.x * PF_BLOCK + threadIdx.x;
    if (r >= n_pad) return;
    const int32_t i = perm[r];
    dst_new[r] = i >= 0 ? src_old[i] : 0.0;
}

__global__ __launch_bounds__(PF_BLOCK) void k_permute_out(const double* __restrict__ ws, int64_t n_pad, int32_t first,
                                                          int32_t count, const int32_t* __restrict__ iperm, int64_t n,
                                                          double* __restrict__ dst_old ) {
    const int64_t i = (int64_t)blockIdx.x * PF_BLOCK + threadIdx.x;
    if (i >= n) return;
    const int64_t r = iperm[i];
    for (int c = 0; c < count; ++c) dst_old[(int64_t)c * n + i] = ws[(int64_t)(first + c) * n_pad + r];
}

__global__ __launch_bounds__(PF_BLOCK) void k_null_vector(double* __restrict__ x, const int32_t* __restrict__ label,
                                                          const int32_t* __restrict__ rowptr,
                                                          const double* __restrict__ deg, const int32_t* __restrict__ perm,
                                                          int64_t n_pad, int32_t root, int32_t sym) {
    const int64_t r = (int64_t)blockIdx.x * PF_BLOCK + threadIdx.x;
    if (r >= n_pad) return;
    const int32_t i = perm[r];
    double v = 0.0;
    if (i >= 0 && label[i] == root && rowptr[i + 1] > rowptr[i]) v = sym ? sqrt(deg[i] + 1e-8) : 1.0;
    x[r] = v;
}

constexpr int COMBINE_COLS = 8;
__global__ __launch_bounds__(PF_BLOCK) void k_combine(double* __restrict__ ws, int64_t n_pad, int32_t src_first, int32_t m,
                                                      const double* __restrict__ Y, int32_t k, int32_t c0, int32_t ncols,
                                                      int32_t dst_first, int32_t src_first2, int32_t dst_first2) {
    const int64_t i = (int64_t)blockIdx.x * PF_BLOCK + threadIdx.x;
    if (i >= n_pad) return;
    if (blockIdx.y) src_first = src_first2, dst_first = dst_first2;
    double acc[COMBINE_COLS];
#pragma unroll
    for (int c = 0; c < COMBINE_COLS; ++c) acc[c] = 0.0;
    for (int b = 0; b < m; ++b) {
        const double v = ws[(int64_t)(src_first + b) * n_pad + i];
        const double* yr = Y + (int64_t)b * k + c0;
#pragma unroll
        for (int c = 0; c < COMBINE_COLS; ++c)
            if (c < ncols) acc[c] += v * yr[c];
    }
#pragma unroll
    for (int c = 0; c < COMBINE_COLS; ++c)
        if (c < ncols) ws[(int64_t)(dst_first + c0 + c) * n_pad + i] = acc[c];
}

__global__ __launch_bounds__(PF_BLOCK) void k_resnorm_partial(const double* __restrict__ ax, const double* __restrict__ x,
                                                              double lam, int64_t n_pad, int64_t n_chunks,
                                                              double* __restrict__ partial) {
    __shared__ double red[PF_BLOCK / PF_WAVE];
    const int64_t lo = (int64_t)blockIdx.x * PF_DOT_CHUNK;
    const int64_t hi = lo + PF_DOT_CHUNK < n_pad ? lo + PF_DOT_CHUNK : n_pad;
    double s = 0.0;
    for (int64_t i = lo + threadIdx.x; i < hi; i += PF_BLOCK) {
        const double r = ax[i] - lam * x[i];
        s += r * r;
    }
#pragma unroll
    for (int off = PF_WAVE / 2; off > 0; off >>= 1) s += __shfl_down(s, off, PF_WAVE);
    if ((threadIdx.x & (PF_WAVE - 1)) == 0) red[threadIdx.x / PF_WAVE] = s;
    __syncthreads();
    if (threadIdx.x == 0) partial[blockIdx.x] = (red[0] + red[1]) + (red[2] + red[3]);
}

__global__ __launch_bounds__(PF_BLOCK) void k_gram_partial(const double* __restrict__ ws, int64_t n_pad, int32_t first_a, int32_t first_b,
                                                           int32_t count_b, int64_t n_chunks, double* __restrict__ partial) {
    __shared__ double red[PF_BLOCK / PF_WAVE];
    const int p = blockIdx.y;
    const int i = p / count_b, j = p - i * count_b;
    const double* v = ws + (int64_t)(first_b + j) * n_pad;
    const double* w = ws + (int64_t)(first_a + i) * n_pad;
    const int64_t lo = (int64_t)blockIdx.x * PF_DOT_CHUNK;
    const int64_t hi = lo + PF_DOT_CHUNK < n_pad ? lo + PF_DOT_CHUNK : n_pad;
    double s = 0.0;
    for (int64_t r = lo + 2 * threadIdx.x; r < hi; r += 2 * PF_BLOCK) {
        const double2 a = *reinterpret_cast<const double2*>(v + r);
        const double2 c = *reinterpret_cast<const double2*>(w + r);
        s += a.x * c.x;
        s += a.y * c.y;
    }
#pragma unroll
    for (int off = PF_WAVE / 2; off > 0; off >>= 1) s += __shfl_down(s, off, PF_WAVE);
    if ((threadIdx.x & (PF_WAVE - 1)) == 0) red[threadIdx.x / PF_WAVE] = s;
    __syncthreads();
    if (threadIdx.x == 0) partial[(int64_t)p * n_chunks + blockIdx.x] = (red[0] + red[1]) + (red[2] + red[3]);
}

constexpr int PF_RESNORMS_MAX = 64;
struct LamArgs {
    double lam[PF_RESNORMS_MAX];
};
__global__ __launch_bounds__(PF_BLOCK) void k_resnorms_partial(const double* __restrict__ ws, int64_t n_pad, int32_t ax_first,
                                                               int32_t x_first, LamArgs la, int64_t n_chunks,
                                                               double* __restrict__ partial) {
    __shared__ double red[PF_BLOCK / PF_WAVE];
    const int b = blockIdx.y;
    const double* ax = ws + (int64_t)(ax_first + b) * n_pad;
    const double* x = ws + (int64_t)(x_first + b) * n_pad;
    const double lam = la.lam[b];
    const int64_t lo = (int64_t)blockIdx.x * PF_DOT_CHUNK;
    const int64_t hi = lo + PF_DOT_CHUNK < n_pad ? lo + PF_DOT_CHUNK : n_pad;
    double s = 0.0;
    for (int64_t i = lo + threadIdx.x; i < hi; i += PF_BLOCK) {
        const double r = ax[i] - lam * x[i];
        s += r * r;
    }
#pragma unroll
    for (int off = PF_WAVE / 2; off > 0; off >>= 1) s += __shfl_down(s, off, PF_WAVE);
    if ((threadIdx.x & (PF_WAVE - 1)) == 0) red[threadIdx.x / PF_WAVE] = s;
    __syncthreads();
    if (threadIdx.x == 0) partial[(int64_t)b * n_chunks + blockIdx.x] = (red[0] + red[1]) + (red[2] + red[3]);
}

struct VecStats {
    double sumsq, vmin, vmax, absmax, at_absmax;
    int64_t arg;
};

__device__ __forceinline__ void stats_merge(VecStats& a, const VecStats& b) {
    a.sumsq += b.sumsq;
    a.vmin = fmin(a.vmin, b.vmin);
    a.vmax = fmax(a.vmax, b.vmax);
    if (b.absmax > a.absmax || (b.absmax == a.absmax && b.arg < a.arg)) {
        a.absmax = b.absmax;
        a.at_absmax = b.at_absmax;
        a.arg = b.arg;
    }
}

__device__ __forceinline__ VecStats stats_shfl(const VecStats& v, int off) {
    VecStats o;
    o.sumsq = __shfl_down(v.sumsq, off, PF_WAVE);
    o.vmin = __shfl_down(v.vmin, off, PF_WAVE);
    o.vmax = __shfl_down(v.vmax, off, PF_WAVE);
    o.absmax = __shfl_down(v.absmax, off, PF_WAVE);
    o.at_absmax = __shfl_down(v.at_absmax, off, PF_WAVE);
    o.arg = __shfl_down(v.arg, off, PF_WAVE);
    return o;
}

__global__ __launch_bounds__(PF_BLOCK) void k_vec_stats_partial(const double* __restrict__ ws, int64_t n_pad, int64_t n,
                                                                int32_t first, const double* __restrict__ sg,
                                                                const int32_t* __restrict__ perm, const int32_t* __restrict__ perm_m,
                                                                int32_t from_sym, int64_t n_chunks, VecStats* __restrict__ partial) {
    __shared__ VecStats red[PF_BLOCK / PF_WAVE];
    const int b = blockIdx.y;
    const double* x = ws + (int64_t)(first + b) * n_pad;
    const int64_t lo = (int64_t)blockIdx.x * PF_DOT_CHUNK;
    const int64_t hi0 = lo + PF_DOT_CHUNK;
    const int64_t hi = hi0 < n ? hi0 : n;
    VecStats st{0.0, INFINITY, -INFINITY, -1.0, 0.0, (int64_t)1 << 62};
    for (int64_t r = lo + threadIdx.x; r < hi; r += PF_BLOCK) {
        const int64_t i = perm[r];
        double v = x[r];
        if (from_sym) v *= sg[perm_m[r]];
        VecStats e{v * v, v, v, fabs(v), v, i};
        stats_merge(st, e);
    }
#pragma unroll
    for (int off = PF_WAVE / 2; off > 0; off >>= 1) {
        VecStats o = stats_shfl(st, off);
        stats_merge(st, o);
    }
    if ((threadIdx.x & (PF_WAVE - 1)) == 0) red[threadIdx.x / PF_WAVE] = st;
    __syncthreads();
    if (threadIdx.x == 0) {
        VecStats t = red[0];
        stats_merge(t, red[1]);
        stats_merge(t, red[2]);
        stats_merge(t, red[3]);
        partial[(int64_t)b * n_chunks + blockIdx.x] = t;
    }
}

__global__ __launch_bounds__(PF_WAVE) void k_vec_stats_finish(const VecStats* __restrict__ partial, int64_t n_chunks,
                                                              VecStats* __restrict__ out) {
    const int b = blockIdx.x;
    VecStats st{0.0, INFINITY, -INFINITY, -1.0, 0.0, (int64_t)1 << 62};
    for (int64_t k = threadIdx.x; k < n_chunks; k += PF_WAVE) stats_merge(st, partial[(int64_t)b * n_chunks + k]);
#pragma unroll
    for (int off = PF_WAVE / 2; off > 0; off >>= 1) {
        VecStats o = stats_shfl(st, off);
        stats_merge(st, o);
    }
    if (threadIdx.x == 0) out[b] = st;
}

__global__ void k_vec_params(const VecStats* __restrict__ fin, int32_t count, int32_t minmax, double* __restrict__ params) {
    for (int c = threadIdx.x; c < count; c += blockDim.x) {
        const VecStats s = fin[c];
        const double sgn = s.at_absmax < 0.0 ? -1.0 : 1.0;
        const double scale = sgn / sqrt(s.sumsq);
        const double vmin = (sgn > 0 ? s.vmin : s.vmax) * scale;
        const double vmax = (sgn > 0 ? s.vmax : s.vmin) * scale;
        params[4 * c + 0] = scale;
        params[4 * c + 1] = minmax ? vmin : 0.0;
        params[4 * c + 2] = minmax ? (vmax - vmin) : 0.0;
        params[4 * c + 3] = minmax ? 0.5 : 0.0;
    }
}

__global__ __launch_bounds__(PF_BLOCK) void k_vec_apply(const double* __restrict__ ws, int64_t n_pad, int64_t n,
                                                        int32_t first, int32_t count, const double* __restrict__ sg,
                                                        const int32_t* __restrict__ iperm, const int32_t* __restrict__ mrank,
                                                        int32_t from_sym, const double* __restrict__ params, double* __restrict__ out) {
    const int64_t i = (int64_t)blockIdx.x * PF_BLOCK + threadIdx.x;
    if (i >= n) return;
    const int64_t r = iperm[i];
    const double s = from_sym ? sg[mrank ? mrank[i] : i] : 1.0;
    for (int c = 0; c < count; ++c) {
        const double scale = params[4 * c + 0], off = params[4 * c + 1], ptp = params[4 * c + 2], half = params[4 * c + 3];
        double v = (ws[(int64_t)(first + c) * n_pad + r] * s) * scale;
        if (ptp != 0.0) v = (v - off) / ptp - half;
        out[i * count + c] = v;
    }
}

__global__ __launch_bounds__(PF_BLOCK) void k_final_rows(const double* __restrict__ fin, const int64_t* __restrict__ rows, int64_t n_rows,
                                                         int32_t fc, double* __restrict__ out) {
    const int64_t e = (int64_t)blockIdx.x * PF_BLOCK + threadIdx.x;
    if (e >= n_rows * fc) return;
    const int64_t t = e / fc;
    out[e] = fin[rows[t] * fc + (e - t * fc)];
}

__global__ __launch_bounds__(PF_BLOCK) void k_fill_mean_filter(const int32_t* __restrict__ rowptr, const int32_t* __restrict__ col,
                                                               const double* __restrict__ w, const double* __restrict__ deg,
                                                               const int32_t* __restrict__ perm, const int32_t* __restrict__ iperm,
                                                               const int32_t* __restrict__ key, int64_t n_pad,
                                                               const int64_t* __restrict__ slice_ptr,
                                                               int32_t* __restrict__ mf_col, double* __restrict__ mf_val) {
    const int64_t row = (int64_t)blockIdx.x * PF_BLOCK + threadIdx.x;
    if (row >= n_pad) return;
    const int64_t s = row / PF_WAVE;
    const int lane = (int)(row & (PF_WAVE - 1));
    const int32_t width = (int32_t)((slice_ptr[s + 1] - slice_ptr[s]) / PF_WAVE) + 1;
    const int64_t base = slice_ptr[s] + (int64_t)PF_WAVE * s;
    const int32_t i = perm[row];
    int32_t e = 0;
    if (i >= 0) {
        const double dinv = 1.0 / (1.0 + deg[i]);
        bool diag_done = false;
        const int32_t ki = key ? key[i] : i;
        for (int32_t a = rowptr[i + 1] - 1; a >= rowptr[i]; --a) {
            const int32_t j = col[a];
            if (!diag_done && (key ? key[j] : j) < ki) {
                mf_col[base + (int64_t)PF_WAVE * e + lane] = (int32_t)row;
                mf_val[base + (int64_t)PF_WAVE * e + lane] = dinv;
                ++e;
                diag_done = true;
            }
            mf_col[base + (int64_t)PF_WAVE * e + lane] = iperm[j];
            mf_val[base + (int64_t)PF_WAVE * e + lane] = dinv * w[a];
            ++e;
        }
        if (!diag_done) {
            mf_col[base + (int64_t)PF_WAVE * e + lane] = (int32_t)row;
            mf_val[base + (int64_t)PF_WAVE * e + lane] = dinv;
            ++e;
        }
    }
    for (; e < width; ++e) {
        mf_col[base + (int64_t)PF_WAVE * e + lane] = (int32_t)row;
        mf_val[base + (int64_t)PF_WAVE * e + lane] = 0.0;
    }
}

template <int NC>
__global__ __launch_bounds__(PF_BLOCK) void k_mean_filter(const int64_t* __restrict__ slice_ptr, const int32_t* __restrict__ mf_col,
                                                          const double* __restrict__ mf_val, const int32_t* __restrict__ perm,
                                                          int64_t n_pad, int32_t ncols, const double* __restrict__ in,
                                                          double* __restrict__ out) {
    const int64_t row = (int64_t)blockIdx.x * PF_BLOCK + threadIdx.x;
    if (row >= n_pad) return;
    const int64_t s = row / PF_WAVE;
    const int lane = (int)(row & (PF_WAVE - 1));
    const int32_t width = (int32_t)((slice_ptr[s + 1] - slice_ptr[s]) / PF_WAVE) + 1;
    const int64_t base = slice_ptr[s] + (int64_t)PF_WAVE * s + lane;
    const bool real = perm[row] >= 0;
    if constexpr (NC > 0) {
        double acc[NC];
#pragma unroll
        for (int c = 0; c < NC; ++c) acc[c] = 0.0;
        for (int32_t e = 0; e < width; ++e) {
            const int64_t j = mf_col[base + (int64_t)PF_WAVE * e];
            const double v = mf_val[base + (int64_t)PF_WAVE * e];
            if (v != 0.0 || j != row) {
#pragma unroll
                for (int c = 0; c < NC; ++c) acc[c] += v * in[j * NC + c];
            }
        }
#pragma unroll
        for (int c = 0; c < NC; ++c) out[row * NC + c] = real ? acc[c] : 0.0;
    } else {
        for (int32_t c = 0; c < ncols; ++c) {
            double acc = 0.0;
            for (int32_t e = 0; e < width; ++e) {
                const double v = mf_val[base + (int64_t)PF_WAVE * e];
                const int64_t j = mf_col[base + (int64_t)PF_WAVE * e];
                if (v != 0.0 || j != row) acc += v * in[j * ncols + c];
            }
            out[row * ncols + c] = real ? acc : 0.0;
        }
    }
}

__global__ __launch_bounds__(PF_BLOCK) void k_rows_in(const double* __restrict__ src, const int32_t* __restrict__ perm, int64_t n_pad,
                                                      int32_t ncols, double* __restrict__ dst) {
    const int64_t t = (int64_t)blockIdx.x * PF_BLOCK + threadIdx.x;
    if (t >= n_pad * ncols) return;
    const int64_t row = t / ncols;
    const int32_t old = perm[row];
    dst[t] = old >= 0 ? src[(int64_t)old * ncols + (t - row * ncols)] : 0.0;
}
__global__ __launch_bounds__(PF_BLOCK) void k_rows_out(const double* __restrict__ src, const int32_t* __restrict__ iperm, int64_t n,
                                                       int32_t ncols, double* __restrict__ dst) {
    const int64_t t = (int64_t)blockIdx.x * PF_BLOCK + threadIdx.x;
    if (t >= n * ncols) return;
    const int64_t old = t / ncols;
    dst[t] = src[(int64_t)iperm[old] * ncols + (t - old * ncols)];
}

__global__ __launch_bounds__(PF_BLOCK) void k_rows_to_new(const int64_t* __restrict__ old_idx, const int32_t* __restrict__ iperm,
                                                          int64_t cnt, int32_t* __restrict__ new_idx) {
    const int64_t t = (int64_t)blockIdx.x * PF_BLOCK + threadIdx.x;
    if (t < cnt) new_idx[t] = iperm[old_idx[t]];
}
__global__ __launch_bounds__(PF_BLOCK) void k_rows_gather(const double* __restrict__ x, const int32_t* __restrict__ idx, int64_t cnt,
                                                          double* __restrict__ out) {
    const int64_t t = (int64_t)blockIdx.x * PF_BLOCK + threadIdx.x;
    if (t < cnt) out[t] = x[idx[t]];
}
__global__ __launch_bounds__(PF_BLOCK) void k_rows_scatter(double* __restrict__ x, const int32_t* __restrict__ idx, int64_t cnt,
                                                           const double* __restrict__ in) {
    const int64_t t = (int64_t)blockIdx.x * PF_BLOCK + threadIdx.x;
    if (t < cnt) x[idx[t]] = in[t];
}
__global__ __launch_bounds__(PF_BLOCK) void k_rows_gather2(const double* __restrict__ xa, const double* __restrict__ xb,
                                                           const int32_t* __restrict__ idx, int64_t cnt, int64_t stride,
                                                           double* __restrict__ out) {
    const int64_t t = (int64_t)blockIdx.x * PF_BLOCK + threadIdx.x;
    if (t >= cnt) return;
    const int32_t r = idx[t];
    out[t] = xa[r];
    if (xb) out[stride + t] = xb[r];
}
__global__ __launch_bounds__(PF_BLOCK) void k_rows_scatter2(double* __restrict__ xa, double* __restrict__ xb,
                                                            const int32_t* __restrict__ idx, const int64_t* __restrict__ off,
                                                            int64_t cnt, int64_t stride, const double* __restrict__ src) {
    const int64_t t = (int64_t)blockIdx.x * PF_BLOCK + threadIdx.x;
    if (t >= cnt) return;
    const int32_t r = idx[t];
    const int64_t o = off[t];
    xa[r] = src[o];
    if (xb) xb[r] = src[o + stride];
}
__global__ __launch_bounds__(PF_BLOCK) void k_rows_fill(double* __restrict__ x, const int32_t* __restrict__ idx, int64_t cnt,
                                                        double value) {
    const int64_t t = (int64_t)blockIdx.x * PF_BLOCK + threadIdx.x;
    if (t < cnt) x[idx[t]] = value;
}

int stage_ensure(pf_graph* g, int64_t elems) {
    if (elems <= g->stage_cap) return PF_OK;
    pf_free(g->ctx->stream, g->stage);
    g->stage = nullptr;
    g->stage_cap = 0;
    PF_HIP(pf_malloc(g->ctx->stream, (void**)&g->stage, sizeof(double) * (size_t)elems));
    g->stage_cap = elems;
    return PF_OK;
}

int check_slots(pf_graph* g, int32_t first, int32_t count, const char* who) {
    PF_CHECK(g != nullptr, PF_E_ARG, "%s: graph is NULL", who);
    PF_HIP(hipSetDevice(g->ctx->device));
    PF_CHECK(first >= 0 && count >= 0 && first + count <= g->n_slots, PF_E_ARG, "%s: slots [%d,%d) outside workspace of %d",
             who, first, first + count, g->n_slots);
    return PF_OK;
}

const double* op_values(pf_graph* g, int32_t op) {
    if (op == PF_OP_RW) return g->sval_rw;
    if (op == PF_OP_SYM) return g->sval_sym;
    return nullptr;
}

OpArgs op_args(pf_graph* g, const double* vals, const double* x, const double* prev, double* out, double alpha, double shift,
               double beta) {
    return OpArgs{g->slice_ptr, g->scol, vals, g->diag, x, prev, out, alpha, shift, beta, (unsigned)(g->n_pad / PF_OP_BLOCK)};
}

int64_t op_bytes(const pf_graph* g) {
    return 12 * (g->nnz_w + g->n - g->n_isolated) + 20 * g->n + 4;
}

int launch_op(pf_graph* g, const double* vals, const double* x, const double* prev, double* out, double alpha, double shift,
              double beta) {
    hipStream_t st = g->ctx->stream;
    const OpArgs a = op_args(g, vals, x, prev, out, alpha, shift, beta);
    if (prev)
        k_sell_op<true><<<a.n_blocks, PF_OP_BLOCK, 0, st>>>(a);
    else
        k_sell_op<false><<<a.n_blocks, PF_OP_BLOCK, 0, st>>>(a);
    PF_HIP(hipGetLastError());
    return PF_OK;
}

int launch_op2(pf_graph* ga, const OpArgs& a, const OpArgs& b, bool has_prev) {
    hipStream_t st = ga->ctx->stream;
    if (has_prev)
        k_sell_op2<true><<<a.n_blocks + b.n_blocks, PF_OP_BLOCK, 0, st>>>(a, b);
    else
        k_sell_op2<false><<<a.n_blocks + b.n_blocks, PF_OP_BLOCK, 0, st>>>(a, b);
    PF_HIP(hipGetLastError());
    return PF_OK;
}

struct ChebRun {
    pf_graph* g;
    const double* vals;
    const double* src;
    double* dst;
    int32_t degree;
    double c, e, rho;
    const double* yp = nullptr;
    const double* yc = nullptr;
    int32_t done = 0;

    int32_t left() const { return degree - done; }
    double* free_tmp(int which) const {
        for (int t = 0; t < PF_WS_TMPS; ++t) {
            double* b = pf_tmp(g, t);
            if (b != yp && b != yc && which-- == 0) return b;
        }
        return nullptr;
    }
    OpArgs first() {
        double* target = degree == 1 ? dst : pf_tmp(g, 0);
        const OpArgs a = op_args(g, vals, src, nullptr, target, 1.0 / (e * rho), c, 0.0);
        yp = src, yc = target, done = 1;
        return a;
    }
    OpArgs single() {
        double* target = left() == 1 ? dst : free_tmp(0);
        const OpArgs a = op_args(g, vals, yc, yp, target, 2.0 / (e * rho), c, 1.0 / (rho * rho));
        yp = yc, yc = target, done += 1;
        return a;
    }
};

struct OpTimer {
    pf_ctx* c;
    int64_t launches;
    double bytes;
    bool on;
    int64_t persist_steps = 0;
    double lds_bytes = 0.0;
    hipEvent_t e0 = nullptr, e1 = nullptr;
    OpTimer(pf_ctx* ctx, int64_t n, double b) : c(ctx), launches(n), bytes(b), on(ctx->timing) {
        if (on && ctx->timing_stride > 1) on = (ctx->timing_count++ % ctx->timing_stride) == 0;
        if (!on) return;
        if (c->spans_pending.size() >= 4096) (void)pf_timing_collect(c);
        if (!c->spans_free.empty()) {
            e0 = c->spans_free.back().first;
            e1 = c->spans_free.back().second;
            c->spans_free.pop_back();
        } else if (hipEventCreate(&e0) != hipSuccess || hipEventCreate(&e1) != hipSuccess) {
            on = false;
            return;
        }
        hipEventRecord(e0, c->stream);
    }
    int finish() {
        if (!on) return PF_OK;
        PF_HIP(hipEventRecord(e1, c->stream));
        c->spans_pending.push_back({e0, e1, launches, bytes, persist_steps, lds_bytes});
        return PF_OK;
    }
};

int small_to_host(pf_graph* g, const double* d_src, double* out, size_t count) {
    pf_ctx* c = g->ctx;
    hipStream_t st = c->stream;
    const size_t bytes = sizeof(double) * count;
    void* pin = nullptr;
    if (bytes <= ((size_t)1 << 16) && pf_pinned_scratch(c, bytes, &pin) == PF_OK) {
        PF_TRY(pf_copy_by_kernel(st, d_src, pin, bytes));
        PF_HIP(hipStreamSynchronize(st));
        memcpy(out, pin, bytes);
        return PF_OK;
    }
    PF_HIP(hipMemcpyAsync(out, d_src, bytes, hipMemcpyDeviceToHost, st));
    PF_HIP(hipStreamSynchronize(st));
    return PF_OK;
}

int dots_device(pf_graph* g, int32_t w, int32_t first, int32_t count, double* d_out, double* d_acc, int accumulate) {
    hipStream_t st = g->ctx->stream;
    PF_TRY(pf_reduce_ensure(g, count));
    dim3 grid((unsigned)g->n_chunks, (unsigned)count);
    k_dot_partial<<<grid, PF_BLOCK, 0, st>>>(g->ws, g->n_pad, first, w, g->n_chunks, g->partials);
    PF_HIP(hipGetLastError());
    k_dot_finish<<<(unsigned)count, PF_WAVE, 0, st>>>(g->partials, g->n_chunks, d_out, d_acc, accumulate);
    PF_HIP(hipGetLastError());
    return PF_OK;
}

}

int pf_reduce_ensure(pf_graph* g, int32_t count) {
    if (count > g->partial_cap) {
        pf_free(g->ctx->stream, g->partials);
        g->partials = nullptr;
        const int32_t cap = std::max(count, 64);
        PF_HIP(pf_malloc(g->ctx->stream, (void**)&g->partials, sizeof(VecStats) * (size_t)cap * (size_t)(g->n_chunks + 1)));
        g->partial_cap = cap;
    }
    if (count > g->coef_cap) {
        pf_free(g->ctx->stream, g->coef);
        g->coef = nullptr;
        const int32_t cap = std::max(count, 64);
        PF_HIP(pf_malloc(g->ctx->stream, (void**)&g->coef, sizeof(double) * 8 * (size_t)cap));
        g->coef_cap = cap;
    }
    return PF_OK;
}

extern "C" {

int pf_ws_ensure(pf_graph* g, int32_t n_slots) {
    PF_CHECK(g != nullptr && n_slots > 0, PF_E_ARG, "pf_ws_ensure: bad argument");
    if (n_slots <= g->n_slots) return PF_OK;
    PF_HIP(hipSetDevice(g->ctx->device));
    hipStream_t st = g->ctx->stream;
    double* nw = nullptr;
    const size_t bytes = sizeof(double) * (size_t)(n_slots + PF_WS_TMPS) * (size_t)g->n_pad;
    PF_HIP(pf_malloc(st, (void**)&nw, bytes));
    PF_HIP(hipMemsetAsync(nw, 0, bytes, st));
    if (g->ws && g->n_slots > 0)
        PF_HIP(hipMemcpyAsync(nw, g->ws, sizeof(double) * (size_t)g->n_slots * g->n_pad, hipMemcpyDeviceToDevice, st));
    pf_free(st, g->ws);
    g->ws = nw;
    g->n_slots = n_slots;
    return PF_OK;
}

int pf_ws_upload(pf_graph* g, int32_t slot, const double* x) {
    PF_TRY(check_slots(g, slot, 1, "pf_ws_upload"));
    PF_CHECK(x != nullptr, PF_E_ARG, "pf_ws_upload: x is NULL");
    hipStream_t st = g->ctx->stream;
    PF_TRY(stage_ensure(g, g->n));
    PF_HIP(hipMemcpyAsync(g->stage, x, sizeof(double) * g->n, hipMemcpyHostToDevice, st));
    k_permute_in<<<nblk(g->n_pad), PF_BLOCK, 0, st>>>(g->stage, g->perm, g->n_pad, pf_slot(g, slot));
    PF_HIP(hipGetLastError());
    PF_HIP(hipStreamSynchronize(st));
    return PF_OK;
}

int pf_ws_download(pf_graph* g, int32_t first, int32_t count, double* out) {
    PF_TRY(check_slots(g, first, count, "pf_ws_download"));
    PF_CHECK(out != nullptr, PF_E_ARG, "pf_ws_download: out is NULL");
    if (count == 0) return PF_OK;
    hipStream_t st = g->ctx->stream;
    PF_TRY(stage_ensure(g, (int64_t)count * g->n));
    k_permute_out<<<nblk(g->n), PF_BLOCK, 0, st>>>(g->ws, g->n_pad, first, count, g->iperm, g->n, g->stage);
    PF_HIP(hipGetLastError());
    PF_HIP(hipMemcpyAsync(out, g->stage, sizeof(double) * (size_t)count * g->n, hipMemcpyDeviceToHost, st));
    PF_HIP(hipStreamSynchronize(st));
    return pf_persist_check(g->ctx);
}

int pf_ws_copy(pf_graph* g, int32_t src, int32_t dst, int32_t count) {
    PF_TRY(check_slots(g, src, count, "pf_ws_copy"));
    PF_TRY(check_slots(g, dst, count, "pf_ws_copy"));
    PF_CHECK(src + count <= dst || dst + count <= src || src == dst, PF_E_ARG, "pf_ws_copy: overlapping ranges");
    if (src == dst || count == 0) return PF_OK;
    PF_HIP(hipMemcpyAsync(pf_slot(g, dst), pf_slot(g, src), sizeof(double) * (size_t)count * g->n_pad,
                          hipMemcpyDeviceToDevice, g->ctx->stream));
    return PF_OK;
}

int pf_mask_isolated(pf_graph* g, int32_t slot) {
    PF_TRY(check_slots(g, slot, 1, "pf_mask_isolated"));
    if (g->n_isolated == 0) return PF_OK;
    k_mask_isolated<<<nblk(g->n), PF_BLOCK, 0, g->ctx->stream>>>(pf_slot(g, slot), g->rowptr, g->perm_m, g->n);
    PF_HIP(hipGetLastError());
    return PF_OK;
}

int pf_start_vector(pf_graph* g, int32_t slot, uint64_t seed) {
    PF_TRY(check_slots(g, slot, 1, "pf_start_vector"));
    k_start_vector<<<nblk(g->n_pad), PF_BLOCK, 0, g->ctx->stream>>>(pf_slot(g, slot), g->smooth, g->perm, g->perm_m, g->rowptr, g->n_pad,
                                                                    (unsigned long long)seed, 0.5);
    PF_HIP(hipGetLastError());
    return PF_OK;
}

int pf_lock_null_vectors(pf_graph* g, int32_t op, int32_t* n_locked) {
    PF_CHECK(g != nullptr && n_locked != nullptr, PF_E_ARG, "pf_lock_null_vectors: NULL argument");
    PF_HIP(hipSetDevice(g->ctx->device));
    PF_CHECK(op == PF_OP_RW || (op == PF_OP_SYM && g->is_symmetric), PF_E_ARG,
             "pf_lock_null_vectors: operator %d not available (W symmetric: %d)", op, g->is_symmetric);
    const int32_t nc = g->n_components;
    PF_TRY(pf_ws_ensure(g, nc + 1));
    hipStream_t st = g->ctx->stream;
    PF_TRY(pf_reduce_ensure(g, 1));
    for (int32_t c = 0; c < nc; ++c) {
        k_null_vector<<<nblk(g->n_pad), PF_BLOCK, 0, st>>>(pf_slot(g, c), g->label, g->rowptr, g->deg, g->perm_m, g->n_pad,
                                                          g->roots[c], op == PF_OP_SYM && !g->unit_g);
        PF_HIP(hipGetLastError());
        PF_TRY(dots_device(g, c, c, 1, g->coef, nullptr, 0));
        k_scale_rsqrt<<<nblk(g->n_pad), PF_BLOCK, 0, st>>>(pf_slot(g, c), g->n_pad, g->coef);
        PF_HIP(hipGetLastError());
    }
    *n_locked = nc;
    return PF_OK;
}

int pf_spmv(pf_graph* g, int32_t op, int32_t src, int32_t dst) {
    PF_TRY(check_slots(g, src, 1, "pf_spmv"));
    PF_TRY(check_slots(g, dst, 1, "pf_spmv"));
    const double* vals = op_values(g, op);
    PF_CHECK(vals != nullptr && src != dst, PF_E_ARG, "pf_spmv: operator %d unavailable or src == dst", op);
    OpTimer t(g->ctx, 1, (double)op_bytes(g));
    PF_TRY(launch_op(g, vals, pf_slot(g, src), nullptr, pf_slot(g, dst), -1.0, 0.0, 0.0));
    return t.finish();
}

int pf_spmv_multi(pf_graph* g, int32_t op, int32_t src_first, int32_t dst_first, int32_t count) {
    PF_CHECK(count >= 0, PF_E_ARG, "pf_spmv_multi: negative count");
    PF_TRY(check_slots(g, src_first, count, "pf_spmv_multi"));
    PF_TRY(check_slots(g, dst_first, count, "pf_spmv_multi"));
    const double* vals = op_values(g, op);
    PF_CHECK(vals != nullptr && (src_first + count <= dst_first || dst_first + count <= src_first), PF_E_ARG,
             "pf_spmv_multi: operator %d unavailable or the slot ranges overlap", op);
    if (count == 0) return PF_OK;
    OpTimer t(g->ctx, count, (double)count * (double)op_bytes(g));
    {
        const OpArgs a = op_args(g, vals, pf_slot(g, src_first), nullptr, pf_slot(g, dst_first), -1.0, 0.0, 0.0);
        k_sell_op_slots<<<dim3(a.n_blocks, (unsigned)count), PF_OP_BLOCK, 0, g->ctx->stream>>>(a, g->n_pad);
        PF_HIP(hipGetLastError());
    }
    return t.finish();
}

int pf_cheb(pf_graph* g, int32_t op, int32_t src, int32_t dst, int32_t degree, double c, double e, double rho) {
    PF_TRY(check_slots(g, src, 1, "pf_cheb"));
    PF_TRY(check_slots(g, dst, 1, "pf_cheb"));
    const double* vals = op_values(g, op);
    PF_CHECK(vals != nullptr && src != dst, PF_E_ARG, "pf_cheb: operator %d unavailable or src == dst", op);
    PF_CHECK(degree >= 1 && e > 0.0 && rho >= 1.0, PF_E_ARG, "pf_cheb: degree %d / half-width %g / rho %g invalid", degree, e, rho);
    OpTimer t(g->ctx, degree, (double)degree * op_bytes(g));
    {
        const pf_persist_args pa{g, vals, pf_slot(g, src), pf_slot(g, dst), degree, c, e, rho};
        int done = 0;
        PF_TRY(pf_persist_cheb(&pa, nullptr, &done, &t.lds_bytes));
        if (done) {
            t.launches = 1;
            t.persist_steps = degree;
            return t.finish();
        }
    }
    ChebRun r{g, vals, pf_slot(g, src), pf_slot(g, dst), degree, c, e, rho};
    int64_t launches = 1;
    {
        const OpArgs a = r.first();
        PF_TRY(launch_op(g, a.sval, a.x, a.prev, a.out, a.alpha, a.shift, a.beta));
    }
    while (r.left() > 0) {
        const OpArgs a = r.single();
        PF_TRY(launch_op(g, a.sval, a.x, a.prev, a.out, a.alpha, a.shift, a.beta));
        ++launches;
    }
    t.launches = launches;
    return t.finish();
}

int pf_cheb2(pf_graph* ga, int32_t op_a, int32_t src_a, int32_t dst_a, int32_t degree_a, double c_a, double e_a, double rho_a,
             pf_graph* gb, int32_t op_b, int32_t src_b, int32_t dst_b, int32_t degree_b, double c_b, double e_b, double rho_b) {
    PF_TRY(check_slots(ga, src_a, 1, "pf_cheb2"));
    PF_TRY(check_slots(ga, dst_a, 1, "pf_cheb2"));
    PF_TRY(check_slots(gb, src_b, 1, "pf_cheb2"));
    PF_TRY(check_slots(gb, dst_b, 1, "pf_cheb2"));
    PF_CHECK(ga != gb && ga->ctx == gb->ctx, PF_E_ARG, "pf_cheb2: the two graphs must differ and share one ctx (stream)");
    const double* va = op_values(ga, op_a);
    const double* vb = op_values(gb, op_b);
    PF_CHECK(va && vb && src_a != dst_a && src_b != dst_b, PF_E_ARG, "pf_cheb2: operator unavailable or src == dst");
    PF_CHECK(degree_a >= 1 && degree_b >= 1 && e_a > 0.0 && e_b > 0.0 && rho_a >= 1.0 && rho_b >= 1.0, PF_E_ARG,
             "pf_cheb2: bad degree / half-width / rho");
    OpTimer t(ga->ctx, std::max(degree_a, degree_b), (double)degree_a * op_bytes(ga) + (double)degree_b * op_bytes(gb));
    {
        const pf_persist_args pa{ga, va, pf_slot(ga, src_a), pf_slot(ga, dst_a), degree_a, c_a, e_a, rho_a};
        const pf_persist_args pb{gb, vb, pf_slot(gb, src_b), pf_slot(gb, dst_b), degree_b, c_b, e_b, rho_b};
        int done = 0;
        PF_TRY(pf_persist_cheb(&pa, &pb, &done, &t.lds_bytes));
        if (done) {
            t.launches = 1;
            t.persist_steps = degree_a + degree_b;
            return t.finish();
        }
        int done_a = 0, done_b = 0;
        PF_TRY(pf_persist_cheb(&pa, nullptr, &done_a, &t.lds_bytes, false));
        PF_TRY(pf_persist_cheb(&pb, nullptr, &done_b, &t.lds_bytes, false));
        if (done_a || done_b) {
            t.launches = done_a + done_b;
            t.persist_steps = (done_a ? degree_a : 0) + (done_b ? degree_b : 0);
            for (int q = 0; q < 2; ++q) {
                if (q == 0 ? done_a : done_b) continue;
                ChebRun r = q == 0 ? ChebRun{ga, va, pf_slot(ga, src_a), pf_slot(ga, dst_a), degree_a, c_a, e_a, rho_a}
                                   : ChebRun{gb, vb, pf_slot(gb, src_b), pf_slot(gb, dst_b), degree_b, c_b, e_b, rho_b};
                OpArgs a = r.first();
                PF_TRY(launch_op(r.g, a.sval, a.x, a.prev, a.out, a.alpha, a.shift, a.beta));
                ++t.launches;
                while (r.left() > 0) {
                    a = r.single();
                    PF_TRY(launch_op(r.g, a.sval, a.x, a.prev, a.out, a.alpha, a.shift, a.beta));
                    ++t.launches;
                }
            }
            return t.finish();
        }
    }
    ChebRun ra{ga, va, pf_slot(ga, src_a), pf_slot(ga, dst_a), degree_a, c_a, e_a, rho_a};
    ChebRun rb{gb, vb, pf_slot(gb, src_b), pf_slot(gb, dst_b), degree_b, c_b, e_b, rho_b};
    int64_t launches = 1;
    {
        const OpArgs a = ra.first(), b = rb.first();
        PF_TRY(launch_op2(ga, a, b, false));
    }
    while (ra.left() > 0 || rb.left() > 0) {
        if (ra.left() > 0 && rb.left() > 0) {
            const OpArgs a = ra.single(), b = rb.single();
            PF_TRY(launch_op2(ga, a, b, true));
        } else {
            ChebRun& r = ra.left() > 0 ? ra : rb;
            const OpArgs a = r.single();
            PF_TRY(launch_op(r.g, a.sval, a.x, a.prev, a.out, a.alpha, a.shift, a.beta));
        }
        ++launches;
    }
    t.launches = launches;
    return t.finish();
}

int pf_orth_cheb2(pf_graph* ga, pf_graph* gb, const int32_t* orth, const int32_t* cheb_i, const double* cheb_d) {
    PF_CHECK(ga && gb && orth && cheb_i && cheb_d, PF_E_ARG, "pf_orth_cheb2: NULL argument");
    PF_TRY(pf_orth_begin2(ga, orth[0], orth[1], orth[2], orth[3], gb, orth[4], orth[5], orth[6], orth[7]));
    return pf_cheb2(ga, cheb_i[0], cheb_i[1], cheb_i[2], cheb_i[3], cheb_d[0], cheb_d[1], cheb_d[2], gb, cheb_i[4], cheb_i[5], cheb_i[6],
                    cheb_i[7], cheb_d[3], cheb_d[4], cheb_d[5]);
}

int pf_dots(pf_graph* g, int32_t w, int32_t first, int32_t count, double* out) {
    PF_TRY(check_slots(g, w, 1, "pf_dots"));
    PF_TRY(check_slots(g, first, count, "pf_dots"));
    PF_CHECK(out != nullptr, PF_E_ARG, "pf_dots: out is NULL");
    if (count == 0) return PF_OK;
    PF_TRY(pf_reduce_ensure(g, count));
    PF_TRY(dots_device(g, w, first, count, g->coef, nullptr, 0));
    return small_to_host(g, g->coef, out, (size_t)count);
}

static std::atomic<int> g_orth_one_launch{-1};

static int64_t orth_local_capacity(int device) {
    static std::mutex m;
// ... 198 lines not shown
        PF_TRY(orth_launch_pass(a2, 2, chunks2, pad2, count2, st));
    }
    ga->orth_wait = ga->orth_ev;
    gb->orth_wait = gb->orth_ev;
    ga->orth_pending = count_a;
    gb->orth_pending = count_b;
    return PF_OK;
}

int pf_orth_end(pf_graph* g, double* h, double* nrm) {
    PF_CHECK(g != nullptr && nrm != nullptr, PF_E_ARG, "pf_orth_end: NULL argument");
    PF_CHECK(g->orth_pending >= 0, PF_E_STATE, "pf_orth_end: no pf_orth_begin in flight");
    const int32_t count = g->orth_pending;
    PF_CHECK(h != nullptr || count == 0, PF_E_ARG, "pf_orth_end: h is NULL");
    PF_HIP(hipSetDevice(g->ctx->device));
    if (g->orth_ticket != 0.0) {
        volatile double* ticket = g->orth_host + count + 2;
        bool got = false;
        for (uint64_t spin = 0;; ++spin) {
            if (__atomic_load_n(reinterpret_cast<volatile uint64_t*>(ticket), __ATOMIC_ACQUIRE) ==
                *reinterpret_cast<const uint64_t*>(&g->orth_ticket)) {
                got = true;
                break;
            }
            if ((spin & 0xfff) == 0xfff) {
                const hipError_t q = hipStreamQuery(g->ctx->stream);
                if (q == hipSuccess) {
                    got = __atomic_load_n(reinterpret_cast<volatile uint64_t*>(ticket), __ATOMIC_ACQUIRE) ==
                          *reinterpret_cast<const uint64_t*>(&g->orth_ticket);
                    break;
                }
                if (q != hipErrorNotReady) {
                    g->orth_pending = -1;
                    PF_HIP(q);
                }
            }
            __builtin_ia32_pause();
        }
        if (!got) {
            g->orth_pending = -1;
            PF_TRY(pf_persist_check(g->ctx));
            PF_CHECK(false, PF_E_HIP, "pf_orth_end: the Gram-Schmidt step never reported (launch failure?)");
        }
    } else {
        PF_HIP(hipEventSynchronize(g->orth_wait));
    }
    g->orth_pending = -1;
    g->orth_redone = 0;
    PF_TRY(pf_persist_check(g->ctx));
    g->orth_twice = g->orth_host[count + 1] == 2.0 ? 1 : 0;
    if (g->orth_host[count + 1] == 1.0) {
        hipStream_t st = g->ctx->stream;
        double* hsum = g->coef + g->coef_cap;
        double* nrm2 = g->coef + 2 * g->coef_cap;
        const int32_t w = g->orth_w, first = g->orth_first;
        const int32_t split = g->orth_split_now >= 0 ? g->orth_split_now : count;
        if (split > 0) {
            k_dot_partial<<<dim3((unsigned)g->n_chunks, (unsigned)split), PF_BLOCK, 0, st>>>(g->ws, g->n_pad, first, w, g->n_chunks, g->partials);
            PF_HIP(hipGetLastError());
        }
        if (count > split) {
            k_dot_partial<<<dim3((unsigned)g->n_chunks, (unsigned)(count - split)), PF_BLOCK, 0, st>>>(g->ws, g->n_pad, g->orth_first2_now, w, g->n_chunks,
                                                                                                   g->partials + (size_t)split * g->n_chunks);
            PF_HIP(hipGetLastError());
        }
        if (split > 0) {
            k_axpy_finishing<<<nblk(g->n_pad / 2), PF_BLOCK, 0, st>>>(g->ws, g->n_pad, first, split, w, g->partials, g->n_chunks, hsum, 1);
            PF_HIP(hipGetLastError());
        }
        if (count > split) {
            k_axpy_finishing<<<nblk(g->n_pad / 2), PF_BLOCK, 0, st>>>(g->ws, g->n_pad, g->orth_first2_now, count - split, w,
                                                                      g->partials + (size_t)split * g->n_chunks, g->n_chunks, hsum + split, 1);
            PF_HIP(hipGetLastError());
        }
        k_dot_partial<<<dim3((unsigned)g->n_chunks, 1u), PF_BLOCK, 0, st>>>(g->ws, g->n_pad, w, w, g->n_chunks, g->partials);
        PF_HIP(hipGetLastError());
        k_scale_finishing<<<nblk(g->n_pad), PF_BLOCK, 0, st>>>(pf_slot(g, w), g->n_pad, g->partials, g->n_chunks, g->orth_normalize,
                                                              hsum, count, nrm2, g->orth_host);
        PF_HIP(hipGetLastError());
        PF_HIP(hipStreamSynchronize(st));
        PF_TRY(pf_persist_check(g->ctx));
        g->orth_redone = 1;
    }
    for (int32_t b = 0; b < count; ++b) h[b] = g->orth_host[b];
    const double v = g->orth_host[count];
    *nrm = sqrt(v > 0.0 ? v : 0.0);
    return PF_OK;
}

int pf_orth_strict(pf_graph* g, int32_t on) {
    PF_CHECK(g != nullptr, PF_E_ARG, "pf_orth_strict: NULL graph");
    g->orth_thresh = on >= 2 ? 4.0 : (on ? 0.5 : 0.09);
    return PF_OK;
}

int pf_orth_device_passes(pf_graph* g, int32_t on) {
    PF_CHECK(g != nullptr, PF_E_ARG, "pf_orth_device_passes: NULL graph");
    g->orth_device_passes = on ? 1 : 0;
    return PF_OK;
}

int pf_orth_one_launch(int32_t on) {
    g_orth_one_launch.store(on < 0 ? -1 : (on ? 1 : 0));
    return PF_OK;
}

int pf_orth_split(pf_graph* g, int32_t first2, int32_t split) {
    PF_CHECK(g != nullptr && split >= 0 && first2 >= 0, PF_E_ARG, "pf_orth_split: bad argument");
    g->orth_split = split;
    g->orth_first2 = first2;
    return PF_OK;
}

int pf_orth_redone(pf_graph* g) {
    PF_CHECK(g != nullptr, PF_E_ARG, "pf_orth_redone: NULL graph");
    return g->orth_redone ? 1 : (g->orth_twice ? 2 : 0);
}

int pf_orth(pf_graph* g, int32_t w, int32_t first, int32_t count, double* h, double* nrm) {
    PF_CHECK(nrm != nullptr && (h != nullptr || count == 0), PF_E_ARG, "pf_orth: NULL output");
    PF_TRY(pf_orth_begin(g, w, first, count, 0));
    return pf_orth_end(g, h, nrm);
}

int pf_scale(pf_graph* g, int32_t slot, double alpha) {
    PF_TRY(check_slots(g, slot, 1, "pf_scale"));
    k_scale<<<nblk(g->n_pad), PF_BLOCK, 0, g->ctx->stream>>>(pf_slot(g, slot), g->n_pad, alpha);
    PF_HIP(hipGetLastError());
    return PF_OK;
}

int pf_combine(pf_graph* g, int32_t src_first, int32_t m, const double* Y, int32_t k, int32_t dst_first) {
    return pf_combine2(g, src_first, m, Y, k, dst_first, -1, -1);
}

}

int pf_combine2(pf_graph* g, int32_t src_first, int32_t m, const double* Y, int32_t k, int32_t dst_first, int32_t src_first2,
                int32_t dst_first2) {
    PF_TRY(check_slots(g, src_first, m, "pf_combine"));
    PF_TRY(check_slots(g, dst_first, k, "pf_combine"));
    PF_CHECK(Y != nullptr && m > 0 && k > 0, PF_E_ARG, "pf_combine: bad argument");
    PF_CHECK(src_first + m <= dst_first || dst_first + k <= src_first, PF_E_ARG, "pf_combine: overlapping ranges");
    const bool two = src_first2 >= 0;
    if (two) {
        PF_TRY(check_slots(g, src_first2, m, "pf_combine"));
        PF_TRY(check_slots(g, dst_first2, k, "pf_combine"));
        PF_CHECK((src_first2 + m <= dst_first2 || dst_first2 + k <= src_first2) && (dst_first + k <= dst_first2 || dst_first2 + k <= dst_first) &&
                     (src_first + m <= dst_first2 || dst_first2 + k <= src_first) && (src_first2 + m <= dst_first || dst_first + k <= src_first2),
                 PF_E_ARG, "pf_combine: overlapping ranges");
    }
    pf_ctx* ctx = g->ctx;
    hipStream_t st = ctx->stream;
    double* dY = nullptr;
    PF_HIP(pf_malloc(st, (void**)&dY, sizeof(double) * (size_t)m * k));
    const size_t bytes = sizeof(double) * (size_t)m * k;
    const void* src = Y;
    bool staged = false;
    if (bytes <= PF_STAGE_BYTES) {
        if (!ctx->stage_ring) {
            if (hipHostMalloc(&ctx->stage_ring, (size_t)PF_STAGE_SLOTS * PF_STAGE_BYTES, hipHostMallocDefault) != hipSuccess) {
                (void)hipGetLastError();
                ctx->stage_ring = nullptr;
            } else {
                for (int i = 0; i < PF_STAGE_SLOTS; ++i) ctx->stage_ev[i] = nullptr;
            }
        }
        if (ctx->stage_ring) {
            const int slot = ctx->stage_next;
            ctx->stage_next = (slot + 1) % PF_STAGE_SLOTS;
            bool ok = true;
            if (!ctx->stage_ev[slot]) ok = hipEventCreateWithFlags(&ctx->stage_ev[slot], hipEventDisableTiming) == hipSuccess;
            else ok = hipEventSynchronize(ctx->stage_ev[slot]) == hipSuccess;
            if (ok) {
                void* dst = static_cast<unsigned char*>(ctx->stage_ring) + (size_t)slot * PF_STAGE_BYTES;
                memcpy(dst, Y, bytes);
                src = dst;
                staged = true;
                hipError_t es = hipMemcpyAsync(dY, src, bytes, hipMemcpyHostToDevice, st);
                if (es == hipSuccess) es = hipEventRecord(ctx->stage_ev[slot], st);
                if (es != hipSuccess) {
                    pf_free(st, dY);
                    PF_HIP(es);
                }
            } else {
                (void)hipGetLastError();
            }
        }
    }
    hipError_t e = staged ? hipSuccess : hipMemcpyAsync(dY, Y, bytes, hipMemcpyHostToDevice, st);
    for (int32_t c0 = 0; c0 < k && e == hipSuccess; c0 += COMBINE_COLS) {
        const int32_t nc = std::min(COMBINE_COLS, k - c0);
        k_combine<<<dim3(nblk(g->n_pad), two ? 2u : 1u), PF_BLOCK, 0, st>>>(g->ws, g->n_pad, src_first, m, dY, k, c0, nc, dst_first, src_first2,
                                                                          dst_first2);
        e = hipGetLastError();
    }
    hipError_t e2 = staged ? hipSuccess : hipStreamSynchronize(st);
    pf_free(st, dY);
    PF_HIP(e);
    PF_HIP(e2);
    return PF_OK;
}

extern "C" {

int pf_resnorm(pf_graph* g, int32_t ax, int32_t x, double lam, double* out) {
    PF_TRY(check_slots(g, ax, 1, "pf_resnorm"));
    PF_TRY(check_slots(g, x, 1, "pf_resnorm"));
    PF_CHECK(out != nullptr, PF_E_ARG, "pf_resnorm: out is NULL");
    hipStream_t st = g->ctx->stream;
    PF_TRY(pf_reduce_ensure(g, 1));
    k_resnorm_partial<<<(unsigned)g->n_chunks, PF_BLOCK, 0, st>>>(pf_slot(g, ax), pf_slot(g, x), lam, g->n_pad, g->n_chunks, g->partials);
    PF_HIP(hipGetLastError());
    k_dot_finish<<<1, PF_WAVE, 0, st>>>(g->partials, g->n_chunks, g->coef, nullptr, 0);
    PF_HIP(hipGetLastError());
    double r2 = 0.0;
    PF_HIP(hipMemcpyAsync(&r2, g->coef, sizeof(double), hipMemcpyDeviceToHost, st));
    PF_HIP(hipStreamSynchronize(st));
    *out = sqrt(r2 > 0.0 ? r2 : 0.0);
    return PF_OK;
}

int pf_gram(pf_graph* g, int32_t first_a, int32_t count_a, int32_t first_b, int32_t count_b, double* out) {
    PF_TRY(check_slots(g, first_a, count_a, "pf_gram"));
    PF_TRY(check_slots(g, first_b, count_b, "pf_gram"));
    PF_CHECK(out != nullptr && count_a > 0 && count_b > 0, PF_E_ARG, "pf_gram: bad argument");
    PF_TRY(pf_reduce_ensure(g, count_a * count_b));
    hipStream_t st = g->ctx->stream;
    k_gram_partial<<<dim3((unsigned)g->n_chunks, (unsigned)(count_a * count_b)), PF_BLOCK, 0, st>>>(g->ws, g->n_pad, first_a, first_b, count_b,
                                                                                                 g->n_chunks, g->partials);
    PF_HIP(hipGetLastError());
    k_dot_finish<<<(unsigned)(count_a * count_b), PF_WAVE, 0, st>>>(g->partials, g->n_chunks, g->coef, nullptr, 0);
    PF_HIP(hipGetLastError());
    return small_to_host(g, g->coef, out, (size_t)count_a * count_b);
}

}

static int small_begin(pf_graph* g, const double* d_src, size_t count, bool root, bool append = false) {
    PF_CHECK(append ? g->small_pending > 0 && !g->small_root && !root : g->small_pending == 0, PF_E_STATE,
             "pf_gram_begin / pf_resnorms_begin: a previous result has not been collected");
    pf_ctx* c = g->ctx;
    hipStream_t st = c->stream;
    const size_t offset = append ? (size_t)g->small_pending : 0;
    if (append) {
        PF_CHECK((int64_t)(offset + count) <= g->small_host_cap, PF_E_STATE, "pf_gram_begin: no room to append");
    } else if ((int64_t)(2 * count) > g->small_host_cap || !g->small_host) {
        if (g->small_host) {
            PF_HIP(hipStreamSynchronize(st));
            c->pinned_pool.emplace_back(g->small_host_cap, g->small_host);
            g->small_host = nullptr;
        }
        const int32_t cap = std::max((int32_t)(2 * count), 128);
        for (size_t i = 0; i < c->pinned_pool.size(); ++i)
            if (c->pinned_pool[i].first >= cap) {
                g->small_host_cap = c->pinned_pool[i].first;
                g->small_host = c->pinned_pool[i].second;
                c->pinned_pool.erase(c->pinned_pool.begin() + (long)i);
                break;
            }
        if (!g->small_host) {
            PF_HIP(hipHostMalloc((void**)&g->small_host, sizeof(double) * (size_t)(cap + 2), hipHostMallocDefault));
            g->small_host_cap = cap;
        }
    }
    if (!g->small_ev) {
        if (!c->event_pool.empty()) {
            g->small_ev = c->event_pool.back();
            c->event_pool.pop_back();
        } else {
            PF_HIP(hipEventCreateWithFlags(&g->small_ev, hipEventDisableTiming));
        }
    }
    PF_TRY(pf_copy_by_kernel(st, d_src, g->small_host + offset, sizeof(double) * count));
    PF_HIP(hipEventRecord(g->small_ev, st));
    g->small_pending = (int32_t)(offset + count);
    g->small_root = root;
    return PF_OK;
}

int pf_small_end(pf_graph* g, double* out) {
    PF_CHECK(g != nullptr && out != nullptr && g->small_pending > 0, PF_E_STATE, "pf_small_end: nothing to collect");
    PF_HIP(hipEventSynchronize(g->small_ev));
    const int32_t count = g->small_pending;
    g->small_pending = 0;
    for (int32_t i = 0; i < count; ++i) {
        const double v = g->small_host[i];
        out[i] = g->small_root ? sqrt(v > 0.0 ? v : 0.0) : v;
    }
    return PF_OK;
}

int pf_gram_begin(pf_graph* g, int32_t first_a, int32_t count_a, int32_t first_b, int32_t count_b, int32_t append) {
    PF_TRY(check_slots(g, first_a, count_a, "pf_gram"));
    PF_TRY(check_slots(g, first_b, count_b, "pf_gram"));
    PF_CHECK(count_a > 0 && count_b > 0, PF_E_ARG, "pf_gram: bad argument");
    PF_TRY(pf_reduce_ensure(g, count_a * count_b));
    hipStream_t st = g->ctx->stream;
    k_gram_partial<<<dim3((unsigned)g->n_chunks, (unsigned)(count_a * count_b)), PF_BLOCK, 0, st>>>(g->ws, g->n_pad, first_a, first_b, count_b,
                                                                                                 g->n_chunks, g->partials);
    PF_HIP(hipGetLastError());
    k_dot_finish<<<(unsigned)(count_a * count_b), PF_WAVE, 0, st>>>(g->partials, g->n_chunks, g->coef, nullptr, 0);
    PF_HIP(hipGetLastError());
    return small_begin(g, g->coef, (size_t)count_a * count_b, false, append != 0);
}

int pf_resnorms_begin(pf_graph* g, int32_t ax_first, int32_t x_first, const double* lam, int32_t count) {
    PF_TRY(check_slots(g, ax_first, count, "pf_resnorms"));
    PF_TRY(check_slots(g, x_first, count, "pf_resnorms"));
    PF_CHECK(lam != nullptr && count > 0, PF_E_ARG, "pf_resnorms: bad argument");
    hipStream_t st = g->ctx->stream;
    PF_TRY(pf_reduce_ensure(g, count));
    for (int32_t at = 0; at < count; at += PF_RESNORMS_MAX) {
        const int32_t nb = std::min(count - at, PF_RESNORMS_MAX);
        LamArgs la{};
        for (int32_t i = 0; i < nb; ++i) la.lam[i] = lam[at + i];
        k_resnorms_partial<<<dim3((unsigned)g->n_chunks, (unsigned)nb), PF_BLOCK, 0, st>>>(g->ws, g->n_pad, ax_first + at, x_first + at, la,
                                                                                        g->n_chunks, g->partials);
        PF_HIP(hipGetLastError());
        k_dot_finish<<<(unsigned)nb, PF_WAVE, 0, st>>>(g->partials, g->n_chunks, g->coef + at, nullptr, 0);
        PF_HIP(hipGetLastError());
    }
    return small_begin(g, g->coef, (size_t)count, true);
}

extern "C" {

int pf_resnorms(pf_graph* g, int32_t ax_first, int32_t x_first, const double* lam, int32_t count, double* out) {
    PF_TRY(check_slots(g, ax_first, count, "pf_resnorms"));
    PF_TRY(check_slots(g, x_first, count, "pf_resnorms"));
    PF_CHECK(out != nullptr && lam != nullptr && count > 0, PF_E_ARG, "pf_resnorms: bad argument");
    hipStream_t st = g->ctx->stream;
    PF_TRY(pf_reduce_ensure(g, count));
    for (int32_t at = 0; at < count; at += PF_RESNORMS_MAX) {
        const int32_t nb = std::min(count - at, PF_RESNORMS_MAX);
        LamArgs la{};
        for (int32_t i = 0; i < nb; ++i) la.lam[i] = lam[at + i];
        k_resnorms_partial<<<dim3((unsigned)g->n_chunks, (unsigned)nb), PF_BLOCK, 0, st>>>(g->ws, g->n_pad, ax_first + at, x_first + at, la,
                                                                                        g->n_chunks, g->partials);
        PF_HIP(hipGetLastError());
        k_dot_finish<<<(unsigned)nb, PF_WAVE, 0, st>>>(g->partials, g->n_chunks, g->coef + at, nullptr, 0);
        PF_HIP(hipGetLastError());
    }
    PF_TRY(small_to_host(g, g->coef, out, (size_t)count));
    for (int32_t i = 0; i < count; ++i) out[i] = sqrt(out[i] > 0.0 ? out[i] : 0.0);
    return PF_OK;
}

static bool downloads_deferred() {
    static const bool on = [] { const char* v = getenv("PF_DOWNLOAD_DEFER"); return !(v && v[0] == '0'); }();
    return on;
}

static int queue_download(pf_graph* g) {
    pf_ctx* ctx = g->ctx;
    const double* src = nullptr;
    {
        std::lock_guard<std::mutex> lk(ctx->deferred_mutex);
        auto it = std::find(ctx->deferred.begin(), ctx->deferred.end(), g);
        if (it != ctx->deferred.end()) ctx->deferred.erase(it);
        src = g->dl_src;
        g->dl_src = nullptr;
    }
    if (!src) return PF_OK;
    PF_HIP(hipEventRecord(g->final_ready, ctx->stream));
    PF_HIP(hipStreamWaitEvent(ctx->copy_stream, g->final_ready, 0));
    PF_HIP(hipMemcpyAsync(g->dl_dst, src, g->dl_bytes, hipMemcpyDeviceToHost, ctx->copy_stream));
    PF_HIP(hipEventRecord(g->final_done, ctx->copy_stream));
    return PF_OK;
}

extern "C++" int pf_download_cancel(pf_graph* g) {
    pf_ctx* ctx = g->ctx;
    bool owed = false;
    {
        std::lock_guard<std::mutex> lk(ctx->deferred_mutex);
        auto it = std::find(ctx->deferred.begin(), ctx->deferred.end(), g);
        if (it != ctx->deferred.end()) ctx->deferred.erase(it);
        owed = g->dl_src != nullptr;
        g->dl_src = nullptr;
    }
    if (g->final_pending != 0) {
        g->final_pending = 0;
        g->final_check = 0;
        if (!owed) (void)hipEventSynchronize(g->final_done);
        pf_free(ctx->stream, g->final_params);
        g->final_params = nullptr;
        pf_free(ctx->stream, g->final_tmp);
        g->final_tmp = nullptr;
    }
    return PF_OK;
}

extern "C++" int pf_downloads_release(pf_ctx* c) {
    for (;;) {
        pf_graph* g = nullptr;
        {
            std::lock_guard<std::mutex> lk(c->deferred_mutex);
            if (c->deferred.empty()) break;
            g = c->deferred.back();
        }
        PF_TRY(queue_download(g));
    }
    return PF_OK;
}

int pf_finalize_vectors_begin(pf_graph* g, int32_t first, int32_t count, int32_t from_sym, int32_t minmax, double* out) {
    PF_TRY(check_slots(g, first, count, "pf_finalize_vectors"));
    PF_CHECK(out != nullptr && count > 0, PF_E_ARG, "pf_finalize_vectors: bad argument");
    PF_CHECK(!from_sym || g->is_symmetric, PF_E_ARG, "pf_finalize_vectors: from_sym on an asymmetric graph");
    PF_TRY(pf_finalize_vectors_end(g));
    pf_ctx* ctx = g->ctx;
    hipStream_t st = ctx->stream;
    if (!ctx->copy_stream) PF_HIP(pf_create_side_stream(&ctx->copy_stream, true));
    for (hipEvent_t* ev : {&g->final_ready, &g->final_done}) {
        if (*ev) continue;
        if (!ctx->event_pool.empty()) {
            *ev = ctx->event_pool.back();
            ctx->event_pool.pop_back();
        } else {
            PF_HIP(hipEventCreateWithFlags(ev, hipEventDisableTiming));
        }
    }
    const int32_t stat_doubles = (int32_t)(sizeof(VecStats) / sizeof(double)) * count;
    if (stat_doubles > g->final_stats_cap + 2 || !g->final_stats) {
        if (g->final_stats) ctx->pinned_pool.emplace_back(g->final_stats_cap, reinterpret_cast<double*>(g->final_stats));
        g->final_stats = nullptr;
        for (size_t i = 0; i < ctx->pinned_pool.size(); ++i)
            if (ctx->pinned_pool[i].first + 2 >= stat_doubles) {
                g->final_stats_cap = ctx->pinned_pool[i].first;
                g->final_stats = ctx->pinned_pool[i].second;
                ctx->pinned_pool.erase(ctx->pinned_pool.begin() + (long)i);
                break;
            }
        if (!g->final_stats) {
            const int32_t cap = std::max(stat_doubles, 384);
            PF_HIP(hipHostMalloc((void**)&g->final_stats, sizeof(double) * (size_t)(cap + 2), hipHostMallocDefault));
            g->final_stats_cap = cap;
        }
    }
    PF_TRY(pf_reduce_ensure(g, count));
    VecStats* part = reinterpret_cast<VecStats*>(g->partials);
    VecStats* fin = part + (size_t)count * g->n_chunks;
    dim3 grid((unsigned)g->n_chunks, (unsigned)count);
    k_vec_stats_partial<<<grid, PF_BLOCK, 0, st>>>(g->ws, g->n_pad, g->n, first, g->sg, g->perm, g->perm_m, from_sym, g->n_chunks, part);
    PF_HIP(hipGetLastError());
    k_vec_stats_finish<<<(unsigned)count, PF_WAVE, 0, st>>>(part, g->n_chunks, fin);
    PF_HIP(hipGetLastError());
    double *d_params = nullptr, *d_out = nullptr;
    pf_free(st, g->final_vecs);
    g->final_vecs = nullptr;
    g->final_count = 0;
    PF_HIP(pf_malloc(st, (void**)&d_params, sizeof(double) * 4 * (size_t)count + sizeof(VecStats) * (size_t)count));
    VecStats* d_stats = reinterpret_cast<VecStats*>(d_params + 4 * (size_t)count);
    hipError_t e = pf_malloc(st, (void**)&d_out, sizeof(double) * (size_t)g->n * count);
    if (e == hipSuccess) {
        k_vec_params<<<1, PF_WAVE, 0, st>>>(fin, count, minmax, d_params);
        k_vec_apply<<<nblk(g->n), PF_BLOCK, 0, st>>>(g->ws, g->n_pad, g->n, first, count, g->sg, g->iperm, g->mrank, from_sym, d_params, d_out);
        e = hipGetLastError();
    }
    if (e == hipSuccess) e = hipMemcpyAsync(d_stats, fin, sizeof(VecStats) * count, hipMemcpyDeviceToDevice, st);
    if (e == hipSuccess) e = hipEventRecord(g->final_ready, st);
    if (e == hipSuccess) e = hipStreamWaitEvent(ctx->copy_stream, g->final_ready, 0);
    if (e == hipSuccess) e = hipMemcpyAsync(g->final_stats, d_stats, sizeof(VecStats) * count, hipMemcpyDeviceToHost, ctx->copy_stream);
    if (e == hipSuccess) e = hipEventRecord(g->final_done, ctx->copy_stream);
    if (e != hipSuccess) {
        (void)hipStreamSynchronize(ctx->copy_stream);
        pf_free(st, d_params);
        pf_free(st, d_out);
        PF_HIP(e);
    }
    g->final_vecs = d_out;
    g->final_count = count;
    g->final_params = d_params;
    g->final_pending = count;
    g->final_check = count;
    g->dl_src = d_out;
    g->dl_dst = out;
    g->dl_bytes = sizeof(double) * (size_t)g->n * count;
    if (downloads_deferred()) {
        std::lock_guard<std::mutex> lk(ctx->deferred_mutex);
        if (std::find(ctx->deferred.begin(), ctx->deferred.end(), g) == ctx->deferred.end()) ctx->deferred.push_back(g);
    } else {
        PF_TRY(queue_download(g));
    }
    return PF_OK;
}

int pf_finalize_vectors_end(pf_graph* g) {
    PF_CHECK(g != nullptr, PF_E_ARG, "pf_finalize_vectors_end: NULL graph");
    if (g->final_pending == 0) return PF_OK;
    g->final_pending = 0;
    const int32_t count = g->final_check;
    g->final_check = 0;
    int rc = queue_download(g);
    const hipError_t e = hipEventSynchronize(g->final_done);
    pf_free(g->ctx->stream, g->final_params);
    g->final_params = nullptr;
    pf_free(g->ctx->stream, g->final_tmp);
    g->final_tmp = nullptr;
    PF_TRY(rc);
    if (count <= 0) {
        PF_HIP(e);
        return PF_OK;
    }
    const VecStats* hs = reinterpret_cast<const VecStats*>(g->final_stats);
    bool sane = e == hipSuccess;
    int32_t bad = 0;
    for (int32_t c = 0; c < count && sane; ++c)
        if (!(hs[c].sumsq > 0.0 && isfinite(hs[c].sumsq))) sane = false, bad = c;
    if (!sane) {
        pf_free(g->ctx->stream, g->final_vecs);
        g->final_vecs = nullptr;
        g->final_count = 0;
    }
    PF_HIP(e);
    PF_CHECK(sane, PF_E_STATE, "pf_finalize_vectors: vector %d has norm^2 %g", bad, hs[(size_t)bad].sumsq);
    return PF_OK;
}

int pf_finalize_vectors(pf_graph* g, int32_t first, int32_t count, int32_t from_sym, int32_t minmax, double* out) {
    PF_TRY(pf_finalize_vectors_begin(g, first, count, from_sym, minmax, out));
    return pf_finalize_vectors_end(g);
}

struct RemapArgs {
    int32_t col[64];
    double sign[64];
};
__global__ __launch_bounds__(PF_BLOCK) void k_final_remap(const double* __restrict__ fin, int64_t n, int32_t fc, int32_t count, RemapArgs m,
                                                          double* __restrict__ out) {
    const int64_t e = (int64_t)blockIdx.x * PF_BLOCK + threadIdx.x;
    if (e >= n * count) return;
    const int64_t i = e / count;
    const int32_t c = (int32_t)(e - i * count);
    out[e] = fin[i * fc + m.col[c]] * m.sign[c];
}

int pf_final_remap_begin(pf_graph* g, const int32_t* col, const double* sign, int32_t count, double* out) {
    PF_CHECK(g && col && sign && out, PF_E_ARG, "pf_final_remap_begin: NULL argument");
    if (!(g->dl_src && g->dl_dst == out)) PF_TRY(pf_finalize_vectors_end(g));
    PF_CHECK(g->final_vecs != nullptr, PF_E_STATE, "pf_final_remap_begin: no pf_finalize_vectors result is resident");
    PF_CHECK(count >= 1 && count <= 64 && count <= g->final_count, PF_E_ARG, "pf_final_remap_begin: count %d out of range", count);
    RemapArgs m{};
    for (int32_t c = 0; c < count; ++c) {
        PF_CHECK(col[c] >= 0 && col[c] < g->final_count, PF_E_ARG, "pf_final_remap_begin: column %d out of range", col[c]);
        m.col[c] = col[c];
        m.sign[c] = sign[c];
    }
    pf_ctx* ctx = g->ctx;
    hipStream_t st = ctx->stream;
    PF_CHECK(ctx->copy_stream && g->final_ready && g->final_done, PF_E_STATE, "pf_final_remap_begin: no download machinery (call after pf_finalize_vectors_begin)");
    double* d_tmp = nullptr;
    PF_HIP(pf_malloc(st, (void**)&d_tmp, sizeof(double) * (size_t)g->n * count));
    k_final_remap<<<nblk(g->n * count), PF_BLOCK, 0, st>>>(g->final_vecs, g->n, g->final_count, count, m, d_tmp);
    const hipError_t e = hipGetLastError();
    if (e != hipSuccess) {
        pf_free(st, d_tmp);
        PF_HIP(e);
    }
    pf_free(st, g->final_tmp);
    g->final_tmp = d_tmp;
    g->dl_src = d_tmp;
    g->dl_dst = out;
    g->dl_bytes = sizeof(double) * (size_t)g->n * count;
    g->final_pending = count;
    if (downloads_deferred()) {
        std::lock_guard<std::mutex> lk(ctx->deferred_mutex);
        if (std::find(ctx->deferred.begin(), ctx->deferred.end(), g) == ctx->deferred.end()) ctx->deferred.push_back(g);
    } else {
        PF_TRY(queue_download(g));
    }
    return PF_OK;
}

static int rows_to_host(pf_graph* g, const double* src, int32_t width, const int64_t* rows, int64_t n_rows, double* out,
                        const char* who) {
    if (n_rows == 0) return PF_OK;
    PF_HIP(hipSetDevice(g->ctx->device));
    hipStream_t st = g->ctx->stream;
    for (int64_t i = 0; i < n_rows; ++i)
        PF_CHECK(rows[i] >= 0 && rows[i] < g->n, PF_E_ARG, "%s: row %lld out of range", who, (long long)rows[i]);
    int64_t* d_rows = nullptr;
    double* d_out = nullptr;
    PF_HIP(pf_malloc(st, (void**)&d_rows, sizeof(int64_t) * n_rows));
    hipError_t e = pf_malloc(st, (void**)&d_out, sizeof(double) * (size_t)n_rows * width);
    if (e == hipSuccess) e = hipMemcpyAsync(d_rows, rows, sizeof(int64_t) * n_rows, hipMemcpyHostToDevice, st);
    if (e == hipSuccess) {
        k_final_rows<<<nblk(n_rows * width), PF_BLOCK, 0, st>>>(src, d_rows, n_rows, width, d_out);
        e = hipGetLastError();
    }
    if (e == hipSuccess) e = hipMemcpyAsync(out, d_out, sizeof(double) * (size_t)n_rows * width, hipMemcpyDeviceToHost, st);
    hipError_t e2 = hipStreamSynchronize(st);
    pf_free(st, d_rows);
    pf_free(st, d_out);
    PF_HIP(e);
    PF_HIP(e2);
    return PF_OK;
}

int pf_final_rows(pf_graph* g, const int64_t* rows, int64_t n_rows, double* out) {
    PF_CHECK(g != nullptr && rows != nullptr && out != nullptr && n_rows >= 0, PF_E_ARG, "pf_final_rows: bad argument");
    PF_CHECK(g->final_vecs != nullptr, PF_E_STATE, "pf_final_rows: no pf_finalize_vectors result is resident");
    return rows_to_host(g, g->final_vecs, g->final_count, rows, n_rows, out, "pf_final_rows");
}

int pf_point_rows(pf_graph* g, const int64_t* rows, int64_t n_rows, double* out) {
    PF_CHECK(g != nullptr && rows != nullptr && out != nullptr && n_rows >= 0, PF_E_ARG, "pf_point_rows: bad argument");
    PF_CHECK(g->pts != nullptr, PF_E_STATE, "pf_point_rows: this graph was not built from a mesh");
    return rows_to_host(g, g->pts, 3, rows, n_rows, out, "pf_point_rows");
}

int pf_spmv_host(pf_graph* g, int32_t op, const double* x, double* y) {
    PF_CHECK(g != nullptr && x != nullptr && y != nullptr, PF_E_ARG, "pf_spmv_host: NULL argument");
// ... 234 lines not shown
```

Measured before the change: 1008.

## Fuse reduction finish into partial kernels via last-block-arrives counters

Gram, residual-norm and vector-stats reductions now have the last arriving block finish the column sum, using an atomic arrival counter and relaxed atomic publishes of the partials. This removes the separate finish kernels and the device-to-pinned copy kernel, since the result is written straight into the pinned host buffer. The self-Gram is merged into the same launch as the cross Gram instead of a second appended call. Null-vector creation now also computes its norm partials, and a small-Y combine variant passes coefficients as kernel arguments. The cost is extra atomics, memory ordering that depends on an s_waitcnt plus relaxed atomics, and direct writes to host memory from inside the kernel.

```diff
diff --git a/include/pyfocusr_hip.h b/include/pyfocusr_hip.h
--- a/include/pyfocusr_hip.h
+++ b/include/pyfocusr_hip.h
@@ -77,6 +77,7 @@
                       double* deg, double* l_diag, int32_t* component_label);
 
 int pf_ws_ensure(pf_graph* g, int32_t n_slots);
+int pf_ws_test_hook(double fill);
 int pf_ws_upload(pf_graph* g, int32_t slot, const double* x);
 int pf_ws_download(pf_graph* g, int32_t first, int32_t count, double* out);
 int pf_ws_copy(pf_graph* g, int32_t src, int32_t dst, int32_t count);
diff --git a/pyfocusr_amd/_hip.py b/pyfocusr_amd/_hip.py
--- a/pyfocusr_amd/_hip.py
+++ b/pyfocusr_amd/_hip.py
@@ -78,6 +78,7 @@
     "pf_graph_get_info": (C.c_int, [C.c_void_p, C.POINTER(GraphInfo)]),
     "pf_graph_download": (C.c_int, [C.c_void_p, _i32p, _i32p, _f64p, _f64p, _f64p, _f64p, _i32p]),
     "pf_ws_ensure": (C.c_int, [C.c_void_p, C.c_int32]),
+    "pf_ws_test_hook": (C.c_int, [C.c_double]),
     "pf_ws_upload": (C.c_int, [C.c_void_p, C.c_int32, _f64p]),
     "pf_ws_download": (C.c_int, [C.c_void_p, C.c_int32, C.c_int32, _f64p]),
     "pf_ws_copy": (C.c_int, [C.c_void_p, C.c_int32, C.c_int32, C.c_int32]),
diff --git a/pyfocusr_amd/csrc/pf_assemble.hip b/pyfocusr_amd/csrc/pf_assemble.hip
--- a/pyfocusr_amd/csrc/pf_assemble.hip
+++ b/pyfocusr_amd/csrc/pf_assemble.hip
@@ -990,6 +990,7 @@
     pf_free(st, g->mf_val);
     pf_free(st, g->ws);
     pf_free(st, g->partials);
+    pf_free(st, g->arrive);
     pf_free(st, g->coef);
     pf_free(st, g->orth_counter);
     if (g->orth_pending >= 0 || g->small_pending > 0 || g->px_state == -2) pfl::sync(st);
diff --git a/pyfocusr_amd/csrc/pf_eigs.hip b/pyfocusr_amd/csrc/pf_eigs.hip
--- a/pyfocusr_amd/csrc/pf_eigs.hip
+++ b/pyfocusr_amd/csrc/pf_eigs.hip
@@ -51,8 +51,7 @@
         return pf_resnorms(g, ax_first, x_first, lam, count, out);
     }
     int gram_begin(int32_t first_a, int32_t count_a, int32_t first_b, int32_t count_b, bool self_b) override {
-        PF_TRY(pf_gram_begin(g, first_a, count_a, first_b, count_b, 0));
-        return self_b ? pf_gram_begin(g, first_b, count_b, first_b, count_b, 1) : PF_OK;
+        return pf_gram_begin(g, first_a, count_a, first_b, count_b, self_b ? 1 : 0);
     }
     bool orth_split(int32_t first2, int32_t split) override { return pf_orth_split(g, first2, split) == PF_OK; }
     int gram_end(double* out) override { return pf_small_end(g, out); }
diff --git a/pyfocusr_amd/csrc/pf_internal.h b/pyfocusr_amd/csrc/pf_internal.h
--- a/pyfocusr_amd/csrc/pf_internal.h
+++ b/pyfocusr_amd/csrc/pf_internal.h
@@ -212,6 +212,7 @@
     int32_t n_slots = 0;
     double* partials = nullptr;
     int32_t partial_cap = 0;
+    unsigned* arrive = nullptr;
     double* coef = nullptr;
     int32_t coef_cap = 0;
     int64_t n_chunks = 0;
@@ -285,7 +286,7 @@
 constexpr int PF_KNN_TREE_MIN_D = 7;
 int pf_knn_tree_run(pf_ctx* c);
 
-int pf_gram_begin(pf_graph* g, int32_t first_a, int32_t count_a, int32_t first_b, int32_t count_b, int32_t append);
+int pf_gram_begin(pf_graph* g, int32_t first_a, int32_t count_a, int32_t first_b, int32_t count_b, int32_t self_b);
 int pf_resnorms_begin(pf_graph* g, int32_t ax_first, int32_t x_first, const double* lam, int32_t count);
 int pf_small_end(pf_graph* g, double* out);
 int pf_combine2(pf_graph* g, int32_t src_first, int32_t m, const double* Y, int32_t k, int32_t dst_first, int32_t src_first2,
diff --git a/pyfocusr_amd/csrc/pf_operator.hip b/pyfocusr_amd/csrc/pf_operator.hip
--- a/pyfocusr_amd/csrc/pf_operator.hip
+++ b/pyfocusr_amd/csrc/pf_operator.hip
@@ -564,22 +564,73 @@
     for (int c = 0; c < count; ++c) dst_old[(int64_t)c * n + i] = ws[(int64_t)(first + c) * n_pad + r];
 }
 
+__device__ __forceinline__ void publish(double* p, double v) {
+    __hip_atomic_store(reinterpret_cast<unsigned long long*>(p), (unsigned long long)__double_as_longlong(v), __ATOMIC_RELAXED,
+                       __HIP_MEMORY_SCOPE_AGENT);
+}
+__device__ __forceinline__ double published(const double* p) {
+    return __longlong_as_double((long long)__hip_atomic_load(reinterpret_cast<const unsigned long long*>(p), __ATOMIC_RELAXED,
+                                                            __HIP_MEMORY_SCOPE_AGENT));
+}
+__device__ __forceinline__ int arrived_last(unsigned* word, unsigned n_blocks) {
+    asm volatile("s_waitcnt vmcnt(0)" ::: "memory");
+    const unsigned seen = __hip_atomic_fetch_add(word, 1u, __ATOMIC_RELAXED, __HIP_MEMORY_SCOPE_AGENT);
+    if (seen + 1u != n_blocks) return 0;
+    __hip_atomic_store(word, 0u, __ATOMIC_RELAXED, __HIP_MEMORY_SCOPE_AGENT);
+    return 1;
+}
+__device__ __forceinline__ double finish_column(const double* partial, int64_t n_chunks) {
+    double s = 0.0;
+    for (int64_t k = threadIdx.x; k < n_chunks; k += PF_WAVE) s += published(partial + k);
+#pragma unroll
+    for (int off = PF_WAVE / 2; off > 0; off >>= 1) s += __shfl_down(s, off, PF_WAVE);
+    return s;
+}
+
 __global__ __launch_bounds__(PF_BLOCK) void k_null_vector(double* __restrict__ x, const int32_t* __restrict__ label,
                                                           const int32_t* __restrict__ rowptr,
                                                           const double* __restrict__ deg, const int32_t* __restrict__ perm,
-                                                          int64_t n_pad, int32_t root, int32_t sym) {
-    const int64_t r = (int64_t)blockIdx.x * PF_BLOCK + threadIdx.x;
-    if (r >= n_pad) return;
-    const int32_t i = perm[r];
-    double v = 0.0;
-    if (i >= 0 && label[i] == root && rowptr[i + 1] > rowptr[i]) v = sym ? sqrt(deg[i] + 1e-8) : 1.0;
-    x[r] = v;
+                                                          int64_t n_pad, int32_t root, int32_t sym, double* __restrict__ partial) {
+    __shared__ double red[PF_BLOCK / PF_WAVE];
+    const int64_t lo = (int64_t)blockIdx.x * PF_DOT_CHUNK;
+    const int64_t hi = lo + PF_DOT_CHUNK < n_pad ? lo + PF_DOT_CHUNK : n_pad;
+    double s = 0.0;
+    for (int64_t r = lo + 2 * threadIdx.x; r < hi; r += 2 * PF_BLOCK) {
+        double2 v;
+        const int32_t i0 = perm[r], i1 = perm[r + 1];
+        v.x = (i0 >= 0 && label[i0] == root && rowptr[i0 + 1] > rowptr[i0]) ? (sym ? sqrt(deg[i0] + 1e-8) : 1.0) : 0.0;
+        v.y = (i1 >= 0 && label[i1] == root && rowptr[i1 + 1] > rowptr[i1]) ? (sym ? sqrt(deg[i1] + 1e-8) : 1.0) : 0.0;
+        *reinterpret_cast<double2*>(x + r) = v;
+        s += v.x * v.x;
+        s += v.y * v.y;
+    }
+#pragma unroll
+    for (int off = PF_WAVE / 2; off > 0; off >>= 1) s += __shfl_down(s, off, PF_WAVE);
+    if ((threadIdx.x & (PF_WAVE - 1)) == 0) red[threadIdx.x / PF_WAVE] = s;
+    __syncthreads();
+    if (threadIdx.x == 0) partial[blockIdx.x] = (red[0] + red[1]) + (red[2] + red[3]);
+}
+
+__global__ __launch_bounds__(PF_BLOCK) void k_scale_by_partials(double* __restrict__ x, int64_t n_pad, const double* __restrict__ partial,
+                                                                int64_t n_chunks) {
+    __shared__ double s_v;
+    if (threadIdx.x < PF_WAVE) {
+        double s = 0.0;
+        for (int64_t k = threadIdx.x; k < n_chunks; k += PF_WAVE) s += partial[k];
+#pragma unroll
+        for (int off = PF_WAVE / 2; off > 0; off >>= 1) s += __shfl_down(s, off, PF_WAVE);
+        if (threadIdx.x == 0) s_v = s;
+    }
+    __syncthreads();
+    const double v = s_v;
+    const int64_t i = (int64_t)blockIdx.x * PF_BLOCK + threadIdx.x;
+    if (i < n_pad && v > 1e-280) x[i] *= 1.0 / sqrt(v);
 }
 
 constexpr int COMBINE_COLS = 8;
-__global__ __launch_bounds__(PF_BLOCK) void k_combine(double* __restrict__ ws, int64_t n_pad, int32_t src_first, int32_t m,
-                                                      const double* __restrict__ Y, int32_t k, int32_t c0, int32_t ncols,
-                                                      int32_t dst_first, int32_t src_first2, int32_t dst_first2) {
+template <class YT>
+__device__ __forceinline__ void combine_rows(double* __restrict__ ws, int64_t n_pad, int32_t src_first, int32_t m, const YT& Y, int32_t k,
+                                             int32_t c0, int32_t ncols, int32_t dst_first, int32_t src_first2, int32_t dst_first2) {
     const int64_t i = (int64_t)blockIdx.x * PF_BLOCK + threadIdx.x;
     if (i >= n_pad) return;
     if (blockIdx.y) src_first = src_first2, dst_first = dst_first2;
@@ -588,14 +639,29 @@
     for (int c = 0; c < COMBINE_COLS; ++c) acc[c] = 0.0;
     for (int b = 0; b < m; ++b) {
         const double v = ws[(int64_t)(src_first + b) * n_pad + i];
-        const double* yr = Y + (int64_t)b * k + c0;
+        const int yr = b * k + c0;
 #pragma unroll
         for (int c = 0; c < COMBINE_COLS; ++c)
-            if (c < ncols) acc[c] += v * yr[c];
+            if (c < ncols) acc[c] += v * Y[yr + c];
     }
 #pragma unroll
     for (int c = 0; c < COMBINE_COLS; ++c)
         if (c < ncols) ws[(int64_t)(dst_first + c0 + c) * n_pad + i] = acc[c];
+}
+__global__ __launch_bounds__(PF_BLOCK) void k_combine(double* __restrict__ ws, int64_t n_pad, int32_t src_first, int32_t m,
+                                                      const double* __restrict__ Y, int32_t k, int32_t c0, int32_t ncols,
+                                                      int32_t dst_first, int32_t src_first2, int32_t dst_first2) {
+    combine_rows(ws, n_pad, src_first, m, Y, k, c0, ncols, dst_first, src_first2, dst_first2);
+}
+constexpr int COMBINE_ARG_DOUBLES = 8 * 49;
+struct CombineY {
+    double y[COMBINE_ARG_DOUBLES];
+    __device__ __forceinline__ double operator[](int i) const { return y[i]; }
+};
+__global__ __launch_bounds__(PF_BLOCK) void k_combine_args(double* __restrict__ ws, int64_t n_pad, int32_t src_first, int32_t m, CombineY Y,
+                                                           int32_t k, int32_t c0, int32_t ncols, int32_t dst_first, int32_t src_first2,
+                                                           int32_t dst_first2) {
+    combine_rows(ws, n_pad, src_first, m, Y, k, c0, ncols, dst_first, src_first2, dst_first2);
 }
 
 __global__ __launch_bounds__(PF_BLOCK) void k_resnorm_partial(const double* __restrict__ ax, const double* __restrict__ x,
@@ -616,13 +682,16 @@
     if (threadIdx.x == 0) partial[blockIdx.x] = (red[0] + red[1]) + (red[2] + red[3]);
 }
 
-__global__ __launch_bounds__(PF_BLOCK) void k_gram_partial(const double* __restrict__ ws, int64_t n_pad, int32_t first_a, int32_t first_b,
-                                                           int32_t count_b, int64_t n_chunks, double* __restrict__ partial) {
+__global__ __launch_bounds__(PF_BLOCK) void k_gram(const double* __restrict__ ws, int64_t n_pad, int32_t first_a, int32_t first_b,
+                                                   int32_t count_b, int32_t n_ab, int64_t n_chunks, double* __restrict__ partial,
+                                                   unsigned* __restrict__ arrive, double* __restrict__ out, double* __restrict__ host_out) {
     __shared__ double red[PF_BLOCK / PF_WAVE];
+    __shared__ int s_last;
     const int p = blockIdx.y;
-    const int i = p / count_b, j = p - i * count_b;
+    const int pl = p < n_ab ? p : p - n_ab;
+    const int i = pl / count_b, j = pl - i * count_b;
     const double* v = ws + (int64_t)(first_b + j) * n_pad;
-    const double* w = ws + (int64_t)(first_a + i) * n_pad;
+    const double* w = ws + (int64_t)((p < n_ab ? first_a : first_b) + i) * n_pad;
     const int64_t lo = (int64_t)blockIdx.x * PF_DOT_CHUNK;
     const int64_t hi = lo + PF_DOT_CHUNK < n_pad ? lo + PF_DOT_CHUNK : n_pad;
     double s = 0.0;
@@ -636,17 +705,28 @@
     for (int off = PF_WAVE / 2; off > 0; off >>= 1) s += __shfl_down(s, off, PF_WAVE);
     if ((threadIdx.x & (PF_WAVE - 1)) == 0) red[threadIdx.x / PF_WAVE] = s;
     __syncthreads();
-    if (threadIdx.x == 0) partial[(int64_t)p * n_chunks + blockIdx.x] = (red[0] + red[1]) + (red[2] + red[3]);
+    if (threadIdx.x == 0) {
+        publish(partial + (int64_t)p * n_chunks + blockIdx.x, (red[0] + red[1]) + (red[2] + red[3]));
+        s_last = arrived_last(arrive + p, (unsigned)n_chunks);
+    }
+    __syncthreads();
+    if (!s_last || threadIdx.x >= PF_WAVE) return;
+    const double sum = finish_column(partial + (int64_t)p * n_chunks, n_chunks);
+    if (threadIdx.x == 0) {
+        out[p] = sum;
+        if (host_out) host_out[p] = sum;
+    }
 }
 
 constexpr int PF_RESNORMS_MAX = 64;
 struct LamArgs {
     double lam[PF_RESNORMS_MAX];
 };
-__global__ __launch_bounds__(PF_BLOCK) void k_resnorms_partial(const double* __restrict__ ws, int64_t n_pad, int32_t ax_first,
-                                                               int32_t x_first, LamArgs la, int64_t n_chunks,
-                                                               double* __restrict__ partial) {
+__global__ __launch_bounds__(PF_BLOCK) void k_resnorms(const double* __restrict__ ws, int64_t n_pad, int32_t ax_first, int32_t x_first,
+                                                       LamArgs la, int64_t n_chunks, double* __restrict__ partial,
+                                                       unsigned* __restrict__ arrive, double* __restrict__ out, double* __restrict__ host_out) {
     __shared__ double red[PF_BLOCK / PF_WAVE];
+    __shared__ int s_last;
     const int b = blockIdx.y;
     const double* ax = ws + (int64_t)(ax_first + b) * n_pad;
     const double* x = ws + (int64_t)(x_first + b) * n_pad;
@@ -662,7 +742,17 @@
     for (int off = PF_WAVE / 2; off > 0; off >>= 1) s += __shfl_down(s, off, PF_WAVE);
     if ((threadIdx.x & (PF_WAVE - 1)) == 0) red[threadIdx.x / PF_WAVE] = s;
     __syncthreads();
-    if (threadIdx.x == 0) partial[(int64_t)b * n_chunks + blockIdx.x] = (red[0] + red[1]) + (red[2] + red[3]);
+    if (threadIdx.x == 0) {
+        publish(partial + (int64_t)b * n_chunks + blockIdx.x, (red[0] + red[1]) + (red[2] + red[3]));
+        s_last = arrived_last(arrive + b, (unsigned)n_chunks);
+    }
+    __syncthreads();
+    if (!s_last || threadIdx.x >= PF_WAVE) return;
+    const double sum = finish_column(partial + (int64_t)b * n_chunks, n_chunks);
+    if (threadIdx.x == 0) {
+        out[b] = sum;
+        if (host_out) host_out[b] = sum;
+    }
 }
 
 struct VecStats {
@@ -692,11 +782,33 @@
     return o;
 }
 
-__global__ __launch_bounds__(PF_BLOCK) void k_vec_stats_partial(const double* __restrict__ ws, int64_t n_pad, int64_t n,
-                                                                int32_t first, const double* __restrict__ sg,
-                                                                const int32_t* __restrict__ perm, const int32_t* __restrict__ perm_m,
-                                                                int32_t from_sym, int64_t n_chunks, VecStats* __restrict__ partial) {
+__device__ __forceinline__ void stats_publish(VecStats* p, const VecStats& v) {
+    publish(&p->sumsq, v.sumsq);
+    publish(&p->vmin, v.vmin);
+    publish(&p->vmax, v.vmax);
+    publish(&p->absmax, v.absmax);
+    publish(&p->at_absmax, v.at_absmax);
+    publish(reinterpret_cast<double*>(&p->arg), __longlong_as_double((long long)v.arg));
+}
+__device__ __forceinline__ VecStats stats_published(const VecStats* p) {
+    VecStats v;
+    v.sumsq = published(&p->sumsq);
+    v.vmin = published(&p->vmin);
+    v.vmax = published(&p->vmax);
+    v.absmax = published(&p->absmax);
+    v.at_absmax = published(&p->at_absmax);
+    v.arg = (int64_t)__double_as_longlong(published(reinterpret_cast<const double*>(&p->arg)));
+    return v;
+}
+
+__global__ __launch_bounds__(PF_BLOCK) void k_vec_stats(const double* __restrict__ ws, int64_t n_pad, int64_t n,
+                                                        int32_t first, const double* __restrict__ sg,
+                                                        const int32_t* __restrict__ perm, const int32_t* __restrict__ perm_m,
+                                                        int32_t from_sym, int64_t n_chunks, VecStats* __restrict__ partial,
+                                                        unsigned* __restrict__ arrive, int32_t minmax, double* __restrict__ params,
+                                                        VecStats* __restrict__ stats_out) {
     __shared__ VecStats red[PF_BLOCK / PF_WAVE];
+    __shared__ int s_last;
     const int b = blockIdx.y;
     const double* x = ws + (int64_t)(first + b) * n_pad;
     const int64_t lo = (int64_t)blockIdx.x * PF_DOT_CHUNK;
@@ -722,34 +834,28 @@
         stats_merge(t, red[1]);
         stats_merge(t, red[2]);
         stats_merge(t, red[3]);
-        partial[(int64_t)b * n_chunks + blockIdx.x] = t;
-    }
-}
-
-__global__ __launch_bounds__(PF_WAVE) void k_vec_stats_finish(const VecStats* __restrict__ partial, int64_t n_chunks,
-                                                              VecStats* __restrict__ out) {
-    const int b = blockIdx.x;
-    VecStats st{0.0, INFINITY, -INFINITY, -1.0, 0.0, (int64_t)1 << 62};
-    for (int64_t k = threadIdx.x; k < n_chunks; k += PF_WAVE) stats_merge(st, partial[(int64_t)b * n_chunks + k]);
+        stats_publish(partial + (int64_t)b * n_chunks + blockIdx.x, t);
+        s_last = arrived_last(arrive + b, (unsigned)n_chunks);
+    }
+    __syncthreads();
+    if (!s_last || threadIdx.x >= PF_WAVE) return;
+    st = VecStats{0.0, INFINITY, -INFINITY, -1.0, 0.0, (int64_t)1 << 62};
+    for (int64_t k = threadIdx.x; k < n_chunks; k += PF_WAVE) stats_merge(st, stats_published(partial + (int64_t)b * n_chunks + k));
 #pragma unroll
     for (int off = PF_WAVE / 2; off > 0; off >>= 1) {
         VecStats o = stats_shfl(st, off);
         stats_merge(st, o);
     }
-    if (threadIdx.x == 0) out[b] = st;
-}
-
-__global__ void k_vec_params(const VecStats* __restrict__ fin, int32_t count, int32_t minmax, double* __restrict__ params) {
-    for (int c = threadIdx.x; c < count; c += blockDim.x) {
-        const VecStats s = fin[c];
-        const double sgn = s.at_absmax < 0.0 ? -1.0 : 1.0;
-        const double scale = sgn / sqrt(s.sumsq);
-        const double vmin = (sgn > 0 ? s.vmin : s.vmax) * scale;
-        const double vmax = (sgn > 0 ? s.vmax : s.vmin) * scale;
-        params[4 * c + 0] = scale;
-        params[4 * c + 1] = minmax ? vmin : 0.0;
-        params[4 * c + 2] = minmax ? (vmax - vmin) : 0.0;
-        params[4 * c + 3] = minmax ? 0.5 : 0.0;
+    if (threadIdx.x == 0) {
+        stats_out[b] = st;
+        const double sgn = st.at_absmax < 0.0 ? -1.0 : 1.0;
+        const double scale = sgn / sqrt(st.sumsq);
+        const double vmin = (sgn > 0 ? st.vmin : st.vmax) * scale;
+        const double vmax = (sgn > 0 ? st.vmax : st.vmin) * scale;
+        params[4 * b + 0] = scale;
+        params[4 * b + 1] = minmax ? vmin : 0.0;
+        params[4 * b + 2] = minmax ? (vmax - vmin) : 0.0;
+        params[4 * b + 3] = minmax ? 0.5 : 0.0;
     }
 }
 
@@ -914,6 +1020,12 @@
     if (t < cnt) x[idx[t]] = value;
 }
 
+std::atomic<double> g_ws_test_fill{0.0};
+__global__ __launch_bounds__(PF_BLOCK) void k_ws_fill(double* __restrict__ x, int64_t count, double value) {
+    const int64_t i = (int64_t)blockIdx.x * PF_BLOCK + threadIdx.x;
+    if (i < count) x[i] = value;
+}
+
 int stage_ensure(pf_graph* g, int64_t elems) {
     if (elems <= g->stage_cap) return PF_OK;
     pf_free(g->ctx->stream, g->stage);
@@ -1067,6 +1179,10 @@
         g->partials = nullptr;
         const int32_t cap = std::max(count, 64);
         PF_HIP(pf_malloc(g->ctx->stream, (void**)&g->partials, sizeof(VecStats) * (size_t)cap * (size_t)(g->n_chunks + 1)));
+        pf_free(g->ctx->stream, g->arrive);
+        g->arrive = nullptr;
+        PF_HIP(pf_malloc(g->ctx->stream, (void**)&g->arrive, sizeof(unsigned) * (size_t)cap));
+        PF_HIP(hipMemsetAsync(g->arrive, 0, sizeof(unsigned) * (size_t)cap, g->ctx->stream));
         g->partial_cap = cap;
     }
     if (count > g->coef_cap) {
@@ -1089,12 +1205,24 @@
     double* nw = nullptr;
     const size_t bytes = sizeof(double) * (size_t)(n_slots + PF_WS_TMPS) * (size_t)g->n_pad;
     PF_HIP(pf_malloc(st, (void**)&nw, bytes));
-    PF_HIP(hipMemsetAsync(nw, 0, bytes, st));
+    if (const double fill = g_ws_test_fill.load()) {
+        const int64_t count = (int64_t)(n_slots + PF_WS_TMPS) * g->n_pad;
+        k_ws_fill<<<nblk(count), PF_BLOCK, 0, st>>>(nw, count, fill);
+        PF_HIP(hipGetLastError());
+    }
+    if (g->n_pad > g->n)
+        PF_HIP(hipMemset2DAsync(nw + g->n, sizeof(double) * (size_t)g->n_pad, 0, sizeof(double) * (size_t)(g->n_pad - g->n),
+                                (size_t)(n_slots + PF_WS_TMPS), st));
     if (g->ws && g->n_slots > 0)
         PF_HIP(hipMemcpyAsync(nw, g->ws, sizeof(double) * (size_t)g->n_slots * g->n_pad, hipMemcpyDeviceToDevice, st));
     pf_free(st, g->ws);
     g->ws = nw;
     g->n_slots = n_slots;
+    return PF_OK;
+}
+
+int pf_ws_test_hook(double fill) {
+    g_ws_test_fill.store(fill);
     return PF_OK;
 }
 
@@ -1159,11 +1287,10 @@
     hipStream_t st = g->ctx->stream;
     PF_TRY(pf_reduce_ensure(g, 1));
     for (int32_t c = 0; c < nc; ++c) {
-        k_null_vector<<<nblk(g->n_pad), PF_BLOCK, 0, st>>>(pf_slot(g, c), g->label, g->rowptr, g->deg, g->perm_m, g->n_pad,
-                                                          g->roots[c], op == PF_OP_SYM && !g->unit_g);
+        k_null_vector<<<(unsigned)g->n_chunks, PF_BLOCK, 0, st>>>(pf_slot(g, c), g->label, g->rowptr, g->deg, g->perm_m, g->n_pad, g->roots[c],
+                                                                 op == PF_OP_SYM && !g->unit_g, g->partials);
         PF_HIP(hipGetLastError());
-        PF_TRY(dots_device(g, c, c, 1, g->coef, nullptr, 0));
-        k_scale_rsqrt<<<nblk(g->n_pad), PF_BLOCK, 0, st>>>(pf_slot(g, c), g->n_pad, g->coef);
+        k_scale_by_partials<<<nblk(g->n_pad), PF_BLOCK, 0, st>>>(pf_slot(g, c), g->n_pad, g->partials, g->n_chunks);
         PF_HIP(hipGetLastError());
     }
     *n_locked = nc;
@@ -1668,6 +1795,17 @@
     }
     pf_ctx* ctx = g->ctx;
     hipStream_t st = ctx->stream;
+    if ((int64_t)m * k <= COMBINE_ARG_DOUBLES) {
+        CombineY ya;
+        memcpy(ya.y, Y, sizeof(double) * (size_t)m * k);
+        for (int32_t c0 = 0; c0 < k; c0 += COMBINE_COLS) {
+            const int32_t nc = std::min(COMBINE_COLS, k - c0);
+            k_combine_args<<<dim3(nblk(g->n_pad), two ? 2u : 1u), PF_BLOCK, 0, st>>>(g->ws, g->n_pad, src_first, m, ya, k, c0, nc, dst_first,
+                                                                                   src_first2, dst_first2);
+            PF_HIP(hipGetLastError());
+        }
+        return PF_OK;
+    }
     double* dY = nullptr;
     PF_HIP(pf_malloc(st, (void**)&dY, sizeof(double) * (size_t)m * k));
     const size_t bytes = sizeof(double) * (size_t)m * k;
@@ -1743,31 +1881,25 @@
     PF_CHECK(out != nullptr && count_a > 0 && count_b > 0, PF_E_ARG, "pf_gram: bad argument");
     PF_TRY(pf_reduce_ensure(g, count_a * count_b));
     hipStream_t st = g->ctx->stream;
-    k_gram_partial<<<dim3((unsigned)g->n_chunks, (unsigned)(count_a * count_b)), PF_BLOCK, 0, st>>>(g->ws, g->n_pad, first_a, first_b, count_b,
-                                                                                                 g->n_chunks, g->partials);
-    PF_HIP(hipGetLastError());
-    k_dot_finish<<<(unsigned)(count_a * count_b), PF_WAVE, 0, st>>>(g->partials, g->n_chunks, g->coef, nullptr, 0);
+    k_gram<<<dim3((unsigned)g->n_chunks, (unsigned)(count_a * count_b)), PF_BLOCK, 0, st>>>(g->ws, g->n_pad, first_a, first_b, count_b,
+                                                                                         count_a * count_b, g->n_chunks, g->partials, g->arrive,
+                                                                                         g->coef, nullptr);
     PF_HIP(hipGetLastError());
     return small_to_host(g, g->coef, out, (size_t)count_a * count_b);
 }
 
 }
 
-static int small_begin(pf_graph* g, const double* d_src, size_t count, bool root, bool append = false) {
-    PF_CHECK(append ? g->small_pending > 0 && !g->small_root && !root : g->small_pending == 0, PF_E_STATE,
-             "pf_gram_begin / pf_resnorms_begin: a previous result has not been collected");
+static int small_prepare(pf_graph* g, size_t count, double** host) {
+    PF_CHECK(g->small_pending == 0, PF_E_STATE, "pf_gram_begin / pf_resnorms_begin: a previous result has not been collected");
     pf_ctx* c = g->ctx;
-    hipStream_t st = c->stream;
-    const size_t offset = append ? (size_t)g->small_pending : 0;
-    if (append) {
-        PF_CHECK((int64_t)(offset + count) <= g->small_host_cap, PF_E_STATE, "pf_gram_begin: no room to append");
-    } else if ((int64_t)(2 * count) > g->small_host_cap || !g->small_host) {
+    if ((int64_t)count > g->small_host_cap || !g->small_host) {
         if (g->small_host) {
-            PF_HIP(hipStreamSynchronize(st));
+            PF_HIP(hipStreamSynchronize(c->stream));
             c->pinned_pool.emplace_back(g->small_host_cap, g->small_host);
             g->small_host = nullptr;
         }
-        const int32_t cap = std::max((int32_t)(2 * count), 128);
+        const int32_t cap = std::max((int32_t)count, 128);
         for (size_t i = 0; i < c->pinned_pool.size(); ++i)
             if (c->pinned_pool[i].first >= cap) {
                 g->small_host_cap = c->pinned_pool[i].first;
@@ -1788,9 +1920,13 @@
             PF_HIP(hipEventCreateWithFlags(&g->small_ev, hipEventDisableTiming));
         }
     }
-    PF_TRY(pf_copy_by_kernel(st, d_src, g->small_host + offset, sizeof(double) * count));
-    PF_HIP(hipEventRecord(g->small_ev, st));
-    g->small_pending = (int32_t)(offset + count);
+    *host = g->small_host;
+    return PF_OK;
+}
+
+static int small_queued(pf_graph* g, size_t count, bool root) {
+    PF_HIP(hipEventRecord(g->small_ev, g->ctx->stream));
+    g->small_pending = (int32_t)count;
     g->small_root = root;
     return PF_OK;
 }
@@ -1807,18 +1943,18 @@
     return PF_OK;
 }
 
-int pf_gram_begin(pf_graph* g, int32_t first_a, int32_t count_a, int32_t first_b, int32_t count_b, int32_t append) {
+int pf_gram_begin(pf_graph* g, int32_t first_a, int32_t count_a, int32_t first_b, int32_t count_b, int32_t self_b) {
     PF_TRY(check_slots(g, first_a, count_a, "pf_gram"));
     PF_TRY(check_slots(g, first_b, count_b, "pf_gram"));
     PF_CHECK(count_a > 0 && count_b > 0, PF_E_ARG, "pf_gram: bad argument");
-    PF_TRY(pf_reduce_ensure(g, count_a * count_b));
-    hipStream_t st = g->ctx->stream;
-    k_gram_partial<<<dim3((unsigned)g->n_chunks, (unsigned)(count_a * count_b)), PF_BLOCK, 0, st>>>(g->ws, g->n_pad, first_a, first_b, count_b,
-                                                                                                 g->n_chunks, g->partials);
+    const int32_t n_ab = count_a * count_b, total = n_ab + (self_b ? count_b * count_b : 0);
+    PF_TRY(pf_reduce_ensure(g, total));
+    double* host = nullptr;
+    PF_TRY(small_prepare(g, (size_t)total, &host));
+    k_gram<<<dim3((unsigned)g->n_chunks, (unsigned)total), PF_BLOCK, 0, g->ctx->stream>>>(g->ws, g->n_pad, first_a, first_b, count_b, n_ab,
+                                                                                       g->n_chunks, g->partials, g->arrive, g->coef, host);
     PF_HIP(hipGetLastError());
-    k_dot_finish<<<(unsigned)(count_a * count_b), PF_WAVE, 0, st>>>(g->partials, g->n_chunks, g->coef, nullptr, 0);
-    PF_HIP(hipGetLastError());
-    return small_begin(g, g->coef, (size_t)count_a * count_b, false, append != 0);
+    return small_queued(g, (size_t)total, false);
 }
 
 int pf_resnorms_begin(pf_graph* g, int32_t ax_first, int32_t x_first, const double* lam, int32_t count) {
@@ -1827,17 +1963,18 @@
     PF_CHECK(lam != nullptr && count > 0, PF_E_ARG, "pf_resnorms: bad argument");
     hipStream_t st = g->ctx->stream;
     PF_TRY(pf_reduce_ensure(g, count));
+    double* host = nullptr;
+    PF_TRY(small_prepare(g, (size_t)count, &host));
     for (int32_t at = 0; at < count; at += PF_RESNORMS_MAX) {
         const int32_t nb = std::min(count - at, PF_RESNORMS_MAX);
         LamArgs la{};
         for (int32_t i = 0; i < nb; ++i) la.lam[i] = lam[at + i];
-        k_resnorms_partial<<<dim3((unsigned)g->n_chunks, (unsigned)nb), PF_BLOCK, 0, st>>>(g->ws, g->n_pad, ax_first + at, x_first + at, la,
-                                                                                        g->n_chunks, g->partials);
+        k_resnorms<<<dim3((unsigned)g->n_chunks, (unsigned)nb), PF_BLOCK, 0, st>>>(g->ws, g->n_pad, ax_first + at, x_first + at, la, g->n_chunks,
+                                                                                g->partials + (size_t)at * g->n_chunks, g->arrive + at,
+                                                                                g->coef + at, host + at);
         PF_HIP(hipGetLastError());
-        k_dot_finish<<<(unsigned)nb, PF_WAVE, 0, st>>>(g->partials, g->n_chunks, g->coef + at, nullptr, 0);
-        PF_HIP(hipGetLastError());
-    }
-    return small_begin(g, g->coef, (size_t)count, true);
+    }
+    return small_queued(g, (size_t)count, true);
 }
 
 extern "C" {
@@ -1852,10 +1989,9 @@
         const int32_t nb = std::min(count - at, PF_RESNORMS_MAX);
         LamArgs la{};
         for (int32_t i = 0; i < nb; ++i) la.lam[i] = lam[at + i];
-        k_resnorms_partial<<<dim3((unsigned)g->n_chunks, (unsigned)nb), PF_BLOCK, 0, st>>>(g->ws, g->n_pad, ax_first + at, x_first + at, la,
-                                                                                        g->n_chunks, g->partials);
-        PF_HIP(hipGetLastError());
-        k_dot_finish<<<(unsigned)nb, PF_WAVE, 0, st>>>(g->partials, g->n_chunks, g->coef + at, nullptr, 0);
+        k_resnorms<<<dim3((unsigned)g->n_chunks, (unsigned)nb), PF_BLOCK, 0, st>>>(g->ws, g->n_pad, ax_first + at, x_first + at, la, g->n_chunks,
+                                                                                g->partials + (size_t)at * g->n_chunks, g->arrive + at,
+                                                                                g->coef + at, nullptr);
         PF_HIP(hipGetLastError());
     }
     PF_TRY(small_to_host(g, g->coef, out, (size_t)count));
@@ -1957,12 +2093,7 @@
     }
     PF_TRY(pf_reduce_ensure(g, count));
     VecStats* part = reinterpret_cast<VecStats*>(g->partials);
-    VecStats* fin = part + (size_t)count * g->n_chunks;
     dim3 grid((unsigned)g->n_chunks, (unsigned)count);
-    k_vec_stats_partial<<<grid, PF_BLOCK, 0, st>>>(g->ws, g->n_pad, g->n, first, g->sg, g->perm, g->perm_m, from_sym, g->n_chunks, part);
-    PF_HIP(hipGetLastError());
-    k_vec_stats_finish<<<(unsigned)count, PF_WAVE, 0, st>>>(part, g->n_chunks, fin);
-    PF_HIP(hipGetLastError());
     double *d_params = nullptr, *d_out = nullptr;
     pf_free(st, g->final_vecs);
     g->final_vecs = nullptr;
@@ -1971,11 +2102,11 @@
     VecStats* d_stats = reinterpret_cast<VecStats*>(d_params + 4 * (size_t)count);
     hipError_t e = pf_malloc(st, (void**)&d_out, sizeof(double) * (size_t)g->n * count);
     if (e == hipSuccess) {
-        k_vec_params<<<1, PF_WAVE, 0, st>>>(fin, count, minmax, d_params);
+        k_vec_stats<<<grid, PF_BLOCK, 0, st>>>(g->ws, g->n_pad, g->n, first, g->sg, g->perm, g->perm_m, from_sym, g->n_chunks, part, g->arrive,
+                                               minmax, d_params, d_stats);
         k_vec_apply<<<nblk(g->n), PF_BLOCK, 0, st>>>(g->ws, g->n_pad, g->n, first, count, g->sg, g->iperm, g->mrank, from_sym, d_params, d_out);
         e = hipGetLastError();
     }
-    if (e == hipSuccess) e = hipMemcpyAsync(d_stats, fin, sizeof(VecStats) * count, hipMemcpyDeviceToDevice, st);
     if (e == hipSuccess) e = hipEventRecord(g->final_ready, st);
     if (e == hipSuccess) e = hipStreamWaitEvent(ctx->copy_stream, g->final_ready, 0);
     if (e == hipSuccess) e = hipMemcpyAsync(g->final_stats, d_stats, sizeof(VecStats) * count, hipMemcpyDeviceToHost, ctx->copy_stream);
```

After: 1001. No clear change (-0.7%).
